# abacus-gene/paml

Measured on AMD Instinct MI355X. Metric: site-patterns/sec per lnL eval (codeml M0, 61 states), higher is better.
Workload: dtype f64; 1 GPU; codeml M0 61-state, 16 taxa x 1000000 synthetic codon patterns sharded over the GPUs (BASELINE configs[3]); classes=1, kernel=mfma64_jit, parallelism=pattern-shard x1, RCCL all-reduce inside the engine, patterns_rank0=1000000

## Files before the change

### include/paml_amd.h

```cpp
#ifndef PAML_AMD_H
#define PAML_AMD_H

#ifdef __cplusplus
extern "C" {
#endif

typedef struct paml_amd_engine paml_amd_engine;

enum {
   PAML_AMD_OK = 0,
   PAML_AMD_EINVAL = -1,
   PAML_AMD_ENOMEM = -2,
   PAML_AMD_EHIP = -3,
   PAML_AMD_EUNSUPPORTED = -4,
   PAML_AMD_ENOCONV = -5
};

enum {
   PAML_AMD_KEEP_PARTIALS = 1,
   PAML_AMD_JIT = 2,
   PAML_AMD_SHARD = 4
};

enum { PAML_AMD_EIGEN_UVROOT = 0, PAML_AMD_EIGEN_CIJK = 1, PAML_AMD_EIGEN_K80 = 2, PAML_AMD_EIGEN_JC69LIKE = 3, PAML_AMD_EIGEN_QMAT = 4 };
// ... 10 lines not shown
#define PAML_AMD_COMM_ID_BYTES 128
int paml_amd_shard_bounds(long n_patt_global, int world, int rank, long *first, long *count);
int paml_amd_max_ranks(long n_patt_global);
int paml_amd_comm_unique_id(void *id128);
int paml_amd_comm_init(paml_amd_engine *e, int rank, int world, const void *id128, long n_patt_global, long first_pattern);
int paml_amd_comm_destroy(paml_amd_engine *e);
int paml_amd_comm_info(const paml_amd_engine *e, int *rank, int *world, long *n_patt_global, long *first_pattern, int *chunk);
int paml_amd_comm_library(char *path, int cap);
int paml_amd_comm_stats(paml_amd_engine *e, int enable, int *n, double *exchange_us_mean, double *exchange_us_max,
                        double *lane_wait_us_mean, double *lane_wait_us_max);

int paml_amd_set_stream(paml_amd_engine *e, void *hip_stream);

int paml_amd_set_tips(paml_amd_engine *e, const unsigned char *z, int cleandata, int n_codes, const int *n_chara,
                      const unsigned char *chara_map, const double *weights, const int *gene_off);

int paml_amd_set_tree(paml_amd_engine *e, int n_nodes, int root, const int *sons_ptr, const int *sons,
                      const int *label, const unsigned char *scale_node);

int paml_amd_set_pi(paml_amd_engine *e, int n_pi, const double *pi);

int paml_amd_set_eigen_qrev_batch(paml_amd_engine *e, int n_sets, const int *set_ids, const double *Q, const double *pi, const double *scale);
int paml_amd_set_eigen_qrev_batch_sparse(paml_amd_engine *e, int n_sets, const int *set_ids, int nnz, const int *row, const int *col,
                                         const double *vals, const double *pi, const double *scale);
int paml_amd_set_eigen_warm_start(paml_amd_engine *e, int on, long *n_warm);
int paml_amd_get_eigen(paml_amd_engine *e, int set_id, double *U, double *V, double *Root);
int paml_amd_eigen_counters(paml_amd_engine *e, long *n_decomposed, int *sweeps_last_batch, int cap);

int paml_amd_set_eigen_uvroot(paml_amd_engine *e, int set_id, const double *U, const double *V, const double *Root);
int paml_amd_set_eigen_cijk(paml_amd_engine *e, int set_id, int nR, const double *Cijk, const double *Root);
int paml_amd_set_eigen_k80(paml_amd_engine *e, int set_id, double kappa);
int paml_amd_set_eigen_jc69like(paml_amd_engine *e, int set_id);
int paml_amd_set_eigen_qmat(paml_amd_engine *e, int set_id, const double *Q);

int paml_amd_set_classes(paml_amd_engine *e, int mode, int K, const double *freqK, const double *rate, int n_labels,
                         const int *eigen_of, const double *qfactor);

int paml_amd_set_gene_class_rates(paml_amd_engine *e, const double *rate);

int paml_amd_eval(paml_amd_engine *e, const double *branch, const double *gene_rate, double *lnL, double *lnf,
                  double *fhK);

int paml_amd_eval_device(paml_amd_engine *e, const double *branch, const double *gene_rate, double *d_lnL);
int paml_amd_flush(paml_amd_engine *e);
int paml_amd_eigen_status(paml_amd_engine *e);

int paml_amd_eval_dirty(paml_amd_engine *e, const double *branch, const double *gene_rate, const unsigned char *clean,
                        double *lnL);

int paml_amd_eval_adg(paml_amd_engine *e, const double *branch, const double *gene_rate, const double *MK, const int *pose, int ls,
                      double *lnL);

int paml_amd_beb_grid(paml_amd_engine *e, int n_grid, int n_cls, const double *pcl, const int *iw, const double *w_class,
                      double *ln_fx, double *pr_last, double *mean_w, double *sd_w);

int paml_amd_beb_grid_classes(paml_amd_engine *e, int n_grid, int n_cls, const double *pcl, const int *iw, double *ln_fx, double *post);

int paml_amd_eval_batch(paml_amd_engine *e, int n_batch, const double *branch, const double *gene_rate, const int *eigen_of,
                        const double *qfactor, const double *freqK, const double *rate, double *lnL, double *lnf);

int paml_amd_eval_branch(paml_amd_engine *e, int node_b, int n_t, const double *t, const double *branch,
                         const double *gene_rate, double *lnL, double *dlnL, double *ddlnL);
int paml_amd_branch_counters(const paml_amd_engine *e, long *n_calls, long *n_nodes_recomputed);
long paml_amd_branch_coef_hits(const paml_amd_engine *e);
long paml_amd_branch_refill_kernels(const paml_amd_engine *e);
double paml_amd_branch_kernel_ms(paml_amd_engine *e);
int paml_amd_get_branch_partials(paml_amd_engine *e, double *out, long cap, long *rows, int *cols);

int paml_amd_node_posterior(paml_amd_engine *e, int node, const double *branch, const double *gene_rate, double *post);

int paml_amd_get_pmat(paml_amd_engine *e, int gene, int iclass, int node, double *P);
int paml_amd_get_partials(paml_amd_engine *e, int node, int iclass, double *conP);
int paml_amd_get_scale(paml_amd_engine *e, int node, int iclass, double *scale);
int paml_amd_get_partial_sums(paml_amd_engine *e, double *out, int cap);

int paml_amd_profile(paml_amd_engine *e, int enable);
int paml_amd_profile_read(paml_amd_engine *e, double *ms_pmat, double *ms_prune, double *ms_reduce, long *n_evals);

int paml_amd_counters(const paml_amd_engine *e, long *n_eval, long *n_pmat);

int paml_amd_cherry_tables(const paml_amd_engine *e, long *n_tabulated, long *bytes);
int paml_amd_subtree_tables(const paml_amd_engine *e, long *n_tabulated, int *nodes, long *u, int cap, long *bytes, long *blocks_left, long *n_computed);
int paml_amd_subtree_order(const paml_amd_engine *e, int *in_use, long *n_computed, double *host_seconds);

int paml_amd_debug_program(int n_tips, int n_nodes, int root, const int *sons_ptr, const int *sons,
                           const unsigned char *scale_node, int keep_partials, const unsigned char *clean,
                           int *ops_out, int cap, int *max_stack);

int paml_amd_debug_branch_plan(int n_tips, int n_nodes, int root, const int *sons_ptr, const int *sons, const unsigned char *scale_node,
                               int n_calls, const int *node_b, const double *branch, int *ends_out, int *up_out, unsigned char *clean_out,
                               int *ops_out, int cap);

int paml_amd_debug_code_order(int n_states, int n_codes, const int *n_chara, const unsigned char *chara_map, const unsigned char *z,
                              long nz, int *order_out);

int paml_amd_debug_jit(int n_tips, int n_nodes, int root, const int *sons_ptr, const int *sons,
                       const unsigned char *scale_node, char *text_out, int cap, int compile);

int paml_amd_debug_jit_tables(int n_tips, int n_nodes, int root, const int *sons_ptr, const int *sons, const unsigned char *scale_node,
                              int max_tabs, char *text_out, int cap, int *stream_out, int stream_cap, int *n_stream, int *tabs_out,
                              int tabs_cap);

int paml_amd_debug_subtree_classes(int n_tips, int n_nodes, int root, const int *sons_ptr, const int *sons, const unsigned char *z, long n_patt,
                                   int n_codes, unsigned int *u_out, unsigned int *cls_out);

int paml_amd_debug_subtree_order(int n_keys, const unsigned int *keys, const unsigned int *bound, long n_patt, int largest_first, int as_given,
                                 unsigned int *order_out);

int paml_amd_debug_subtree_select(int n_tips, int n_nodes, int root, const int *sons_ptr, const int *sons, const unsigned char *scale_node, int n_states,
                                  int n_codes, int K, const unsigned char *z, long n_patt, int *sel_out, int cap);

int paml_amd_debug_jit_subtree(int n_tips, int n_nodes, int root, const int *sons_ptr, const int *sons, const unsigned char *scale_node, int n_states,
                               int n_codes, int K, const int *sel, int n_sel, int compile, const char *dir, char *text_out, int cap, int *blocks_left);

int paml_amd_jit_prebuild(int n_states, int n_tips, int n_codes, int K, long n_patt_global, int n_nodes, int root, const int *sons_ptr,
                          const int *sons, const unsigned char *scale_node, const char *dir, char *log_out, int log_cap);

const char *paml_amd_kernel_name(const paml_amd_engine *e);

int paml_amd_compress_patterns(int n_seq, int n_sites, int width, const unsigned char *chars, const int *gene, int *n_patt,
                               int *first_site, double *weights, int *pose);

int paml_amd_rell_replicates(int n_trees, int n_patt, const double *w, const double *lnf, int n_genes, const int *gene_off, int n_rep,
                             unsigned long long seed, double *rep);
void paml_amd_rell_info(int *chunk, int *tree_block, int *last_batches, double *last_kernel_ms);

int paml_amd_simulate(paml_amd_engine *e, const double *branch, const double *gene_rate, long n_sites, long first_site,
                      unsigned long long seed, unsigned replicate,
                      unsigned char *z ,
                      unsigned char *cls , unsigned char *anc );
void paml_amd_simulate_info(int *last_batches, double *last_kernel_ms);

int paml_amd_ancestral_marginal(paml_amd_engine *e, const double *branch, const double *gene_rate,
                                int n_query, const int *nodes ,
                                unsigned char *best   ,
                                double *best_prob     ,
                                double *post          );

int paml_amd_ancestral_joint(paml_amd_engine *e, const double *branch, const double *gene_rate,
                             unsigned char *states ,
                             double *ln_best       );

void paml_amd_ancestral_info(int *last_batches, double *last_kernel_ms);

int paml_amd_gradient(paml_amd_engine *e, const double *branch, const double *gene_rate, double *lnL,
                      double *grad   ,
                      double *lnf    ,
                      double *scores );
void paml_amd_gradient_info(int *last_batches, double *last_kernel_ms);

int paml_amd_model_gradient(paml_amd_engine *e, const double *branch, const double *gene_rate, double *lnL,
                            double *g_eff   ,
                            double *g_freqK ,
                            double *g_pi    ,
                            double *g_A     ,
                            double *W       );
void paml_amd_model_gradient_info(int *last_batches, double *last_kernel_ms);
int paml_amd_model_gradient_segment(void);
int paml_amd_model_gradient_sizes(paml_amd_engine *e, int *n_pi, int *n_eigen);

int paml_amd_nni_scores(paml_amd_engine *e, const double *branch, const double *gene_rate,
                        int n_swaps, const int *swaps ,
                        double *lnL0, double *lnL , double *lnf );
void paml_amd_nni_info(int *last_batches, double *last_kernel_ms);
int paml_amd_nni_list(int n_tips, int n_nodes, int root, const int *sons_ptr, const int *sons, int *swaps , int cap);

int paml_amd_edge_scores(paml_amd_engine *e, const double *branch, const double *gene_rate,
                         int n_rows, const int *rows ,
                         const int *ovr_node , const double *ovr_t ,
                         double *lnL0, double *lnL, double *d1, double *d2 , double *lnf );
void paml_amd_edge_info(int *last_batches, double *last_kernel_ms);
int paml_amd_edge_list(int n_tips, int n_nodes, int root, const int *sons_ptr, const int *sons,
                       int *edges , int *five , int cap);

int paml_amd_placement_scores(paml_amd_engine *e, const double *branch, const double *gene_rate,
                              int n_q, const unsigned char *qz ,
                              int n_edges, const int *edges ,
                              int n_pend, const double *pendant , double phi, int pendant_label,
                              double *lnL0, double *lnL , double *lnf );
void paml_amd_placement_info(int *last_batches, double *last_kernel_ms);

int paml_amd_spr_scores(paml_amd_engine *e, const double *branch, const double *gene_rate,
                        int n_moves, const int *moves , double phi,
                        double *lnL0, double *lnL , double *lnf );
void paml_amd_spr_info(int *last_batches, double *last_kernel_ms);
int paml_amd_spr_list(int n_tips, int n_nodes, int root, const int *sons_ptr, const int *sons, int radius, int *moves , int cap);

typedef struct paml_amd_pairset paml_amd_pairset;
int paml_amd_pairset_create(paml_amd_engine *e, paml_amd_pairset **out, int n_pairs, const int *seq_a, const int *seq_b);
void paml_amd_pairset_destroy(paml_amd_pairset *ps);
// ... 13 lines not shown
```

### paml_amd/csrc/device_common.h

```cpp
#pragma once
#ifndef __HIPCC_RTC__
#include <hip/hip_runtime.h>
#endif

#include "../../include/paml_amd.h"

namespace paml_amd {

typedef double v4d __attribute__((ext_vector_type(4)));

enum OpCode : int {
   OP_INIT_ONES = 0, OP_INIT_TIP = 1, OP_MUL_TIP = 2, OP_PUSH = 3, OP_MATMUL = 4, OP_MATMUL_POP = 5,
   OP_SCALE = 6, OP_STORE = 7, OP_LOAD = 8, OP_ROOT = 9, OP_END = 10,
   OP_SET_TIP = 11,
   OP_SET_TIP2 = 12,
   OP_MUL_TIP2 = 13,
   OP_EXPORT = 14
};

struct Op { int code, a, b, c; };
__host__ __device__ inline int mm_pop_slot(const Op &o) { return (o.b & 0xff) - 1; }
__host__ __device__ inline int mm_push_slot(const Op &o) { return ((o.b >> 8) & 0xff) - 1; }


struct PruneArgs {
   const Op *ops;
   const unsigned char *z;
   long z_stride;
   const int2 *tiles;
   int n_tiles;
   const int *gene_off;
   const double *weights;
   int n, n_tips, n_nodes, K, n_genes, n_codes, cleandata, n_pi, mode, n_scale, keep, n_patt;
   const double *pi;
   const double *pint;
   const double *ptip;
   double *fhK;
   double *partials;
   double *scalef;
   double *stack_scratch;
   int stack_overflow_slots;
   int first_matmul;
   int n_int;
   int first_tip;
   const void *stream;
   int n_stream;
   long tip_words;
   double *export_buf;
   double *export_scale;
   unsigned long long *prof;
   int prof_stride, prof_tid;
   const double *pcol;
   double *fscale;
   const unsigned char *ztiles;
   int zt_bytes;
   const unsigned int *zpm;
   int zpm_words;
   int Km;
   int chunk;
   int first_chunk, nb_stride;
   int want_fhk;
   const double *freqK;
   long freqK_bs;
   double *lnf;
   double *red_partial;
   double *red_out;
   int *red_counter;
   int nb_local;
   const int *tile_group0;
   int part_groups;
   double *part_dump;
   const unsigned long long *code_mask;
   const double *ctab;
   int n_ctab;
   const double *stab;
   long stab_rows;
   const int *stab_meta;
   const int *order;
};

__device__ __forceinline__ double root_value(const PruneArgs &a, double f, double lnscale)
{
   if (f <= 0) f = (a.mode == PAML_AMD_MODE_LFUN ? 1e-80 : 1e-300);
   if (a.mode == PAML_AMD_MODE_LFUN || a.n_scale) f = log(f) + lnscale;
   return f;
}


typedef double part2_t __attribute__((ext_vector_type(2)));
__device__ __forceinline__ void part_load(const double *p, int lane, double (&x)[16])
{
   const part2_t *p2 = (const part2_t *)p + lane;
#pragma unroll
   for (int i = 0; i < 8; i++) { const part2_t v = p2[i * 64]; x[2 * i] = v.x; x[2 * i + 1] = v.y; }
}
__device__ __forceinline__ void part_store(double *p, int lane, const double (&x)[16])
{
   part2_t *p2 = (part2_t *)p + lane;
#pragma unroll
   for (int i = 0; i < 8; i++) p2[i * 64] = (part2_t){x[2 * i], x[2 * i + 1]};
}
__host__ __device__ inline int part_index(int m, int lane) { return (((m >> 1) * 64 + lane) << 1) | (m & 1); }

#define MFMA_RS 2
#define MFMA_ZT 128

#define CONST_AS __attribute__((address_space(4)))
template <typename T>
__device__ __forceinline__ const CONST_AS T *as_const(const T *p)
{
   return (const CONST_AS T *)(unsigned long long)p;
}
typedef int v4i __attribute__((ext_vector_type(4)));
__device__ __forceinline__ Op fetch_op(const Op *ops, int ip)
{
   const v4i o = ((const CONST_AS v4i *)(unsigned long long)ops)[ip];
   return Op{o.x, o.y, o.z, o.w};
}

typedef __attribute__((address_space(1))) const void gptr_t;
typedef __attribute__((address_space(3))) void lptr_t;

__device__ __forceinline__ __amdgpu_buffer_rsrc_t make_rsrc(const void *base, unsigned bytes)
{
   return __builtin_amdgcn_make_buffer_rsrc((void *)base, 0, bytes, 0x00020000);
}

__device__ __forceinline__ void dma16(__amdgpu_buffer_rsrc_t r, const void *lds, int voff, int soff)
{
   const unsigned la = (unsigned)(unsigned long long)(__attribute__((address_space(3))) const char *)lds;
   asm volatile("s_mov_b32 m0, %0\n\ts_nop 0\n\tbuffer_load_dwordx4 %1, %2, %3 offen lds"
                :
                : "s"(la), "v"(voff), "s"(r), "s"(soff)
                : "memory", "m0");
}

__device__ __forceinline__ void dma4(__amdgpu_buffer_rsrc_t r, const void *lds, int voff, int soff)
{
   const unsigned la = (unsigned)(unsigned long long)(__attribute__((address_space(3))) const char *)lds;
   asm volatile("s_mov_b32 m0, %0\n\ts_nop 0\n\tbuffer_load_dword %1, %2, %3 offen lds"
                :
                : "s"(la), "v"(voff), "s"(r), "s"(soff)
                : "memory", "m0");
}

template <int WAVES>
__device__ __forceinline__ void stage_p(const double *g, double *s, int wave, int lane)
{
   const __amdgpu_buffer_rsrc_t r = make_rsrc(g, 32768);
#pragma unroll
   for (int c = 0; c < 32 / WAVES; c++) {
      const int chunk = c * WAVES + wave;
      dma16(r, (const char *)s + chunk * 1024, lane * 16, chunk * 1024);
   }
}

__device__ __forceinline__ void mfma_matvec(const double *sPbuf, int lane, const double (&cur)[16], v4d (&acc)[4])
{
   const double2 *sp = (const double2 *)sPbuf;
#pragma unroll
   for (int jb = 0; jb < 4; jb++) acc[jb] = (v4d){0, 0, 0, 0};
// ... 1015 lines not shown
```

### paml_amd/csrc/engine_core.hip

```cpp
#include "engine_state.h"
#include "eigen_kernels.h"

namespace paml_amd {
int launch_eigen_qrev(paml_amd_engine *e, EigenQrevArgs a, int n_sets)
{
   if (!e->eigen_attr_set) {
      for (const void *fn : {(const void *)eigen_qrev_kernel<0>, (const void *)eigen_qrev_kernel<20>, (const void *)eigen_qrev_kernel<60>, (const void *)eigen_qrev_kernel<62>})
         HIPCHK(hipFuncSetAttribute(fn, hipFuncAttributeMaxDynamicSharedMemorySize, (int)EIG_LDS_BYTES));
      e->eigen_attr_set = true;
   }
   static const int sweep_limit = getenv("PAML_AMD_EIGEN_SWEEP_LIMIT") ? std::max(1, atoi(getenv("PAML_AMD_EIGEN_SWEEP_LIMIT"))) : 40;
   a.max_sweeps = sweep_limit;
   const int N_even = (a.n + 1) & ~1;
   if (N_even == 62) hipLaunchKernelGGL(eigen_qrev_kernel<62>, dim3(n_sets), dim3(EIG_NT), EIG_LDS_BYTES, e->stream, a);
   else if (N_even == 60) hipLaunchKernelGGL(eigen_qrev_kernel<60>, dim3(n_sets), dim3(EIG_NT), EIG_LDS_BYTES, e->stream, a);
   else if (N_even == 20) hipLaunchKernelGGL(eigen_qrev_kernel<20>, dim3(n_sets), dim3(EIG_NT), EIG_LDS_BYTES, e->stream, a);
   else hipLaunchKernelGGL(eigen_qrev_kernel<0>, dim3(n_sets), dim3(EIG_NT), EIG_LDS_BYTES, e->stream, a);
   HIPCHK(hipGetLastError());
   return 0;
}
}

extern "C" {

// ... 77 lines not shown
{
   enter(e);
   if (!e) return PAML_AMD_EINVAL;
   (void)hipStreamSynchronize(e->stream);
   e->stream = (hipStream_t)hip_stream;
   return 0;
}

int paml_amd_set_tips(paml_amd_engine *e, const unsigned char *z, int cleandata, int n_codes, const int *n_chara,
                      const unsigned char *chara_map, const double *weights, const int *gene_off)
{
   enter(e);
   if (!e || !z || !weights) return fail(e, PAML_AMD_EINVAL, "set_tips: null argument");
   const int n = e->n;
   std::vector<int> nch;
   std::vector<unsigned char> cmap;
   if (cleandata || !n_chara || !chara_map) {
      if (!cleandata) return fail(e, PAML_AMD_EINVAL, "set_tips: cleandata=0 needs n_chara/chara_map");
      n_codes = n;
      nch.assign(n, 1);
      cmap.assign((size_t)n * n, 0);
      for (int i = 0; i < n; i++) cmap[(size_t)i * n] = (unsigned char)i;
   }
   else {
      if (n_codes < 1 || n_codes > 256) return fail(e, PAML_AMD_EINVAL, "set_tips: n_codes out of range");
      nch.assign(n_chara, n_chara + n_codes);
      cmap.assign(chara_map, chara_map + (size_t)n_codes * n);
      for (int c = 0; c < n_codes; c++) {
         if (nch[c] < 0 || nch[c] > n) return fail(e, PAML_AMD_EINVAL, "set_tips: n_chara out of range");
         unsigned long long seen = 0;
         for (int k = 0; k < nch[c]; k++) {
            const int s = cmap[(size_t)c * n + k];
            if (s >= n) return fail(e, PAML_AMD_EINVAL, "set_tips: chara_map state out of range");
            if ((seen >> s) & 1ull) return fail(e, PAML_AMD_EINVAL, "set_tips: a state listed twice in one code's set");
            seen |= 1ull << s;
         }
      }
   }
   const size_t nz = (size_t)e->n_tips * e->n_patt;
   for (size_t i = 0; i < nz; i++)
      if (z[i] >= n_codes) return fail(e, PAML_AMD_EINVAL, "set_tips: character code >= n_codes");
   std::vector<unsigned char> zperm;
   e->code_nch = nch;
   e->code_new_of.resize(n_codes);
   for (int c = 0; c < n_codes; c++) e->code_new_of[c] = (unsigned char)c;
   if (e->kk == KK_MFMA64 && n_codes > 64) {
      std::vector<long> cnt(n_codes, 0);
      for (size_t i = 0; i < nz; i++) cnt[z[i]]++;
      const std::vector<int> order = code_order(n, n_codes, nch.data(), cmap.data(), cnt.data());
      std::vector<unsigned char> new_of(n_codes);
      std::vector<int> nch2(n_codes);
      std::vector<unsigned char> cmap2((size_t)n_codes * n, 0);
      for (int c = 0; c < n_codes; c++) {
         new_of[order[c]] = (unsigned char)c;
         nch2[c] = nch[order[c]];
         memcpy(&cmap2[(size_t)c * n], &cmap[(size_t)order[c] * n], n);
      }
      nch.swap(nch2);
      cmap.swap(cmap2);
      e->code_new_of = new_of;
      zperm.resize(nz);
      for (size_t i = 0; i < nz; i++) zperm[i] = new_of[z[i]];
      z = zperm.data();
   }
   e->amb_ascending = true;
   for (int c = 64; c < n_codes; c++)
      for (int k = 1; k < nch[c]; k++)
         if (cmap[(size_t)c * n + k] <= cmap[(size_t)c * n + k - 1]) e->amb_ascending = false;
   e->cleandata = cleandata ? 1 : 0;
   e->n_codes = n_codes;
   e->plain_codes = 0;
   while (e->plain_codes < std::min(n, n_codes) && nch[e->plain_codes] == 1 && cmap[(size_t)e->plain_codes * n] == e->plain_codes) e->plain_codes++;
   e->gene_off.assign(e->n_genes + 1, 0);
   if (gene_off) e->gene_off.assign(gene_off, gene_off + e->n_genes + 1);
   else {
      if (e->n_genes != 1) return fail(e, PAML_AMD_EINVAL, "set_tips: gene_off required when n_genes > 1");
      e->gene_off[1] = e->n_patt;
   }
   if (e->gene_off[0] != 0 || e->gene_off[e->n_genes] != e->n_patt)
      return fail(e, PAML_AMD_EINVAL, "set_tips: gene_off must span [0, n_patt]");
   for (int g = 0; g < e->n_genes; g++)
      if (e->gene_off[g + 1] < e->gene_off[g]) return fail(e, PAML_AMD_EINVAL, "set_tips: gene_off must not decrease");
   HIPCHK(upload(e->d_z, z, nz, e->stream));
   if (e->kk == KK_MFMA64 && e->n_genes == 1 && n_codes <= 64) e->h_z.assign(z, z + nz);
   else std::vector<unsigned char>().swap(e->h_z);
   e->tips_gen++;
   HIPCHK(upload(e->d_weights, weights, (size_t)e->n_patt, e->stream));
   HIPCHK(upload(e->d_n_chara, nch.data(), nch.size(), e->stream));
   HIPCHK(upload(e->d_chara_map, cmap.data(), cmap.size(), e->stream));
   HIPCHK(upload(e->d_gene_off, e->gene_off.data(), e->gene_off.size(), e->stream));
   if (e->kk == KK_VALU4 || e->kk == KK_VALU5 || e->kk == KK_VALU20) {
      e->zpm_words = ((e->n_tips + 3) / 4 + 3) / 4 * 4;
      HIPCHK(e->d_zpm.ensure((size_t)e->n_patt * e->zpm_words));
      launch_zpm(e->d_z.p, (long)e->n_patt, e->n_tips, e->n_patt, e->zpm_words, e->d_zpm.p, e->stream);
   }
   HIPCHK(hipStreamSynchronize(e->stream));
   e->tile_stash.built_for = 0;
   int r = build_tiles(e);
   if (r) return r;
   {
      std::vector<unsigned long long> mask(n_codes, 0);
      for (int c = 0; c < n_codes; c++)
         for (int k = 0; k < nch[c]; k++) mask[c] |= 1ull << cmap[(size_t)c * n + k];
      HIPCHK(upload(e->d_code_mask, mask.data(), mask.size(), e->stream));
      HIPCHK(hipStreamSynchronize(e->stream));
   }
   e->have_tips = true;
   e->partials_valid = false;
   e->bl.valid = false;
   return 0;
}

int paml_amd_set_tree(paml_amd_engine *e, int n_nodes, int root, const int *sons_ptr, const int *sons, const int *label,
                      const unsigned char *scale_node)
{
   enter(e);
   if (!e || !sons_ptr || !sons) return fail(e, PAML_AMD_EINVAL, "set_tree: null argument");
   if (n_nodes <= e->n_tips || root < 0 || root >= n_nodes) return fail(e, PAML_AMD_EINVAL, "set_tree: bad sizes");
   TreeDesc t;
   t.n_tips = e->n_tips; t.n_nodes = n_nodes; t.root = root;
   t.sons_ptr.assign(sons_ptr, sons_ptr + n_nodes + 1);
   if (t.sons_ptr[0] != 0) return fail(e, PAML_AMD_EINVAL, "set_tree: sons_ptr[0] != 0");
   for (int i = 0; i < n_nodes; i++)
      if (t.sons_ptr[i + 1] < t.sons_ptr[i]) return fail(e, PAML_AMD_EINVAL, "set_tree: sons_ptr not monotone");
   t.sons.assign(sons, sons + t.sons_ptr[n_nodes]);
   std::vector<int> seen(n_nodes, 0);
   for (int s : t.sons) {
      if (s < 0 || s >= n_nodes || s == root || seen[s]++) return fail(e, PAML_AMD_EINVAL, "set_tree: bad son index");
   }
   for (int i = 0; i < n_nodes; i++) {
      if (i != root && !seen[i]) return fail(e, PAML_AMD_EINVAL, "set_tree: node without father");
      if (i >= e->n_tips && t.is_leaf(i)) return fail(e, PAML_AMD_EINVAL, "set_tree: internal node without sons");
      if (i < e->n_tips && i != root && !t.is_leaf(i)) return fail(e, PAML_AMD_EINVAL, "set_tree: tip with sons");
   }
   t.label.assign(n_nodes, 0);
   if (label) t.label.assign(label, label + n_nodes);
   t.scale_node.assign(n_nodes, 0);
   t.scale_slot.assign(n_nodes, -1);
   if (scale_node) {
      for (int i = 0; i < n_nodes; i++) {
         t.scale_node[i] = scale_node[i] ? 1 : 0;
         if (t.scale_node[i]) t.scale_slot[i] = t.n_scale++;
      }
   }
   std::vector<unsigned char> leaf(n_nodes);
   for (int i = 0; i < n_nodes; i++) leaf[i] = t.is_leaf(i) ? 1 : 0;
   e->tree = std::move(t);
   e->tree_gen++;
   HIPCHK(upload(e->d_label, e->tree.label.data(), e->tree.label.size(), e->stream));
   HIPCHK(upload(e->d_is_leaf, leaf.data(), leaf.size(), e->stream));
   HIPCHK(hipStreamSynchronize(e->stream));
   e->have_tree = true;
   e->pres_valid = false;
   e->prog_valid = false;
   e->partials_valid = false;
   e->bl.valid = false;
   return 0;
}

int paml_amd_set_pi(paml_amd_engine *e, int n_pi, const double *pi)
{
   enter(e);
   if (!e || !pi || (n_pi != 1 && n_pi != e->n_genes)) return fail(e, PAML_AMD_EINVAL, "set_pi: bad arguments");
   const int n = e->n;
   std::vector<double> buf;
   if (e->kk == KK_MFMA64) {
      buf.assign((size_t)n_pi * 64, 0.0);
      for (int g = 0; g < n_pi; g++)
// ... 402 lines not shown
         for (int hl = 0; hl < 16; hl++) {
            const int h = tiles[t].y + w * 16 + hl;
            if (h >= hend) continue;
            const double *grp = raw.data() + (t * MW + w) * 1024;
            for (int j = 0; j < n; j++) conP[(size_t)h * n + j] = grp[part_index(j >> 2, (j & 3) * 16 + hl)];
         }
   }
   return 0;
}

int paml_amd_get_scale(paml_amd_engine *e, int node, int iclass, double *scale)
{
   enter(e);
   if (!e || !scale) return fail(e, PAML_AMD_EINVAL, "get_scale: null argument");
   if (!(e->flags & PAML_AMD_KEEP_PARTIALS) || !e->partials_valid)
      return fail(e, PAML_AMD_EINVAL, "get_scale: needs PAML_AMD_KEEP_PARTIALS and a completed evaluation");
   if (node < 0 || node >= e->tree.n_nodes || iclass < 0 || iclass >= e->K || e->tree.scale_slot[node] < 0)
      return fail(e, PAML_AMD_EINVAL, "get_scale: not a scaling node");
   const double *src = e->d_scalef.p + ((size_t)iclass * e->tree.n_scale + e->tree.scale_slot[node]) * e->n_patt;
   HIPCHK(hipMemcpyAsync(scale, src, (size_t)e->n_patt * sizeof(double), hipMemcpyDeviceToHost, e->stream));
   HIPCHK(hipStreamSynchronize(e->stream));
   return 0;
}

int paml_amd_profile(paml_amd_engine *e, int enable)
{
   if (!e) return PAML_AMD_EINVAL;
   enter(e);
   e->profiling = enable != 0;
   return 0;
}

int paml_amd_profile_read(paml_amd_engine *e, double *ms_pmat, double *ms_prune, double *ms_reduce, long *n_evals)
{
   if (!e) return PAML_AMD_EINVAL;
   HIPCHK(hipStreamSynchronize(e->stream));
   double acc[3] = {0, 0, 0};
   for (size_t i = 0; i + 5 < e->ev_used.size(); i += 6)
      for (int k = 0; k < 3; k++) {
         float ms = 0;
         if (hipEventElapsedTime(&ms, e->ev_used[i + 2 * k], e->ev_used[i + 2 * k + 1]) == hipSuccess) acc[k] += ms;
      }
   for (auto ev : e->ev_used) e->ev_pool.push_back(ev);
   e->ev_used.clear();
   if (ms_pmat) *ms_pmat = acc[0];
   if (ms_prune) *ms_prune = acc[1];
   if (ms_reduce) *ms_reduce = acc[2];
   if (n_evals) *n_evals = e->prof_evals;
   e->prof_evals = 0;
   return 0;
}

int paml_amd_cherry_tables(const paml_amd_engine *e, long *n_tabulated, long *bytes)
{
   if (!e) return PAML_AMD_EINVAL;
   if (n_tabulated) *n_tabulated = e->last_ctab_n;
   if (bytes) *bytes = e->last_ctab_bytes;
   return 0;
}

int paml_amd_subtree_tables(const paml_amd_engine *e, long *n_tabulated, int *nodes, long *u, int cap, long *bytes, long *blocks_left, long *n_computed)
{
   if (!e) return PAML_AMD_EINVAL;
   if (n_tabulated) *n_tabulated = e->last_stab_n;
   for (long i = 0; i < e->last_stab_n && i < cap && i < (long)e->sub.sel.size(); i++) {
      if (nodes) nodes[i] = e->sub.sel[i];
      if (u) u[i] = (long)e->sub.u[e->sub.sel[i]];
   }
   if (bytes) *bytes = e->last_stab_bytes;
   if (blocks_left) *blocks_left = e->last_stab_blocks;
   if (n_computed) *n_computed = e->sub.n_computed;
   return 0;
}

int paml_amd_subtree_order(const paml_amd_engine *e, int *in_use, long *n_computed, double *host_seconds)
{
   if (!e) return PAML_AMD_EINVAL;
   if (in_use) *in_use = (e->last_stab_n && e->sub.ordered) ? 1 : 0;
   if (n_computed) *n_computed = e->sub.n_order_computed;
   if (host_seconds) *host_seconds = e->sub.order_host_s;
   return 0;
}

int paml_amd_counters(const paml_amd_engine *e, long *n_eval, long *n_pmat)
{
   if (!e) return PAML_AMD_EINVAL;
   if (n_eval) *n_eval = e->n_eval;
   if (n_pmat) *n_pmat = e->n_pmat;
   return 0;
}

}
```

### paml_amd/csrc/engine_eval.hip

```cpp
#include "engine_state.h"
#include "kernels_pmat.h"
#include "kernels_prune.h"
#include "kernels_reduce.h"

namespace paml_amd {

int build_tiles(paml_amd_engine *e)
{
   std::vector<int2> tiles;
   for (int g = 0; g < e->n_genes; g++)
      for (int h = e->gene_off[g]; h < e->gene_off[g + 1]; h += e->tile_patt) tiles.push_back(make_int2(g, h));
   e->n_tiles = (int)tiles.size();
   HIPCHK(upload(e->d_tiles, tiles.data(), tiles.size(), e->stream));
   const int tf = e->kk == KK_MFMA64 ? GATHER_WAVES * 16 : 256;
   std::vector<int2> tfull;
   for (int g = 0; g < e->n_genes; g++)
      for (int h = e->gene_off[g]; h < e->gene_off[g + 1]; h += tf) tfull.push_back(make_int2(g, h));
   e->n_tiles_full = (int)tfull.size();
   HIPCHK(upload(e->d_tiles_full, tfull.data(), tfull.size(), e->stream));
   if (e->kk == KK_MFMA64) {
      std::vector<int> g0(tiles.size());
      size_t k = 0;
      int base = 0;
      for (int g = 0; g < e->n_genes; g++) {
// ... 339 lines not shown
      sb.level_first.push_back((int)by_level.size());
      int tiles = 0;
      bool tip_son = false;
      for (int i = 0; i < ns; i++)
         if (sb.sp.sub[i].level == l) {
            by_level.push_back(i);
            tiles = std::max(tiles, (int)((sb.u[sb.sp.sub[i].node] + 127) / 128));
            tip_son = tip_son || sb.sp.sub[i].l.kind == 0 || sb.sp.sub[i].r.kind == 0;
         }
      sb.level_tiles.push_back(tiles);
      sb.level_small.push_back(tip_son ? 0 : 1);
   }
   sb.level_first.push_back((int)by_level.size());
   sb.rowmap.assign(ns, std::vector<unsigned int>());
   std::vector<std::vector<unsigned int>> son_rows(ns);
   for (int i = 0; i < ns; i++) {
      const SubtreeTab &st = sb.sp.sub[i];
      const size_t u = sb.u[st.node];
      const std::vector<unsigned int> &sc = sb.son_cls[st.node];
      std::vector<unsigned int> l(sc.begin(), sc.begin() + u), r(sc.begin() + u, sc.end());
      if (st.l.kind == 2 && !sb.rowmap[st.l.id].empty()) for (unsigned int &x : l) x = sb.rowmap[st.l.id][x];
      if (st.r.kind == 2 && !sb.rowmap[st.r.id].empty()) for (unsigned int &x : r) x = sb.rowmap[st.r.id][x];
      son_rows[i].resize(2 * u);
      if (e->env.subtree_rows) {
         std::vector<unsigned int> by(u);
         for (size_t c = 0; c < u; c++) by[c] = (unsigned int)c;
         std::sort(by.begin(), by.end(), [&](unsigned int a, unsigned int b) { return l[a] != l[b] ? l[a] < l[b] : (r[a] != r[b] ? r[a] < r[b] : a < b); });
         sb.rowmap[i].resize(u);
         for (size_t row = 0; row < u; row++) { sb.rowmap[i][by[row]] = (unsigned int)row; son_rows[i][row] = l[by[row]]; son_rows[i][u + row] = r[by[row]]; }
      }
      else { std::copy(l.begin(), l.end(), son_rows[i].begin()); std::copy(r.begin(), r.end(), son_rows[i].begin() + u); }
   }
   std::vector<SubtreeNodeDev> nodes(ns);
   std::vector<unsigned int> sidx;
   for (int k = 0; k < ns; k++) {
      const SubtreeTab &st = sb.sp.sub[by_level[k]];
      SubtreeNodeDev &nd = nodes[k];
      nd.node = st.node; nd.u = (int)sb.u[st.node]; nd.row0 = row0[by_level[k]];
      nd.lkind = st.l.kind; nd.lid = st.l.kind == 2 ? row0[st.l.id] : st.l.id;
      nd.rkind = st.r.kind; nd.rid = st.r.kind == 2 ? row0[st.r.id] : st.r.id;
      nd.pad = 0;
      nd.sidx = (long)sidx.size();
      sidx.insert(sidx.end(), son_rows[by_level[k]].begin(), son_rows[by_level[k]].end());
   }
   std::vector<int> meta;
   for (int ti : sb.sp.top) { meta.push_back(row0[ti]); meta.push_back((int)sb.u[sb.sp.sub[ti].node]); }
   HIPCHK(upload(sb.d_nodes, nodes.data(), nodes.size(), e->stream));
   HIPCHK(upload(sb.d_sidx, sidx.data(), sidx.size(), e->stream));
   HIPCHK(upload(sb.d_meta, meta.data(), meta.size(), e->stream));
   HIPCHK(hipStreamSynchronize(e->stream));
   return 0;
}

int ensure_subtree_ztiles(paml_amd_engine *e)
{
   paml_amd_engine::Subtree &sb = e->sub;
   if (sb.zt_sel_gen == sb.sel_gen && sb.zt_tiles == e->n_tiles && sb.zt_tile_patt == e->tile_patt) return 0;
   const int n_top = (int)sb.sp.top.size();
   std::vector<unsigned int> top((size_t)n_top * e->n_patt);
   for (int k = 0; k < n_top; k++) {
      const std::vector<unsigned int> &c = sb.cls[sb.sp.sub[sb.sp.top[k]].node], &rm = sb.rowmap[sb.sp.top[k]];
      if (rm.empty()) std::copy(c.begin(), c.end(), top.begin() + (size_t)k * e->n_patt);
      else for (long h = 0; h < e->n_patt; h++) top[(size_t)k * e->n_patt + h] = rm[c[h]];
   }
   sb.ordered = e->env.subtree_order != 0;
   if (sb.ordered && sb.order_sel_gen != sb.sel_gen) {
      const auto t0 = std::chrono::steady_clock::now();
      std::vector<const unsigned int *> keys;
      std::vector<unsigned int> bound;
      for (int k = 0; k < n_top; k++) { keys.push_back(top.data() + (size_t)k * e->n_patt); bound.push_back(sb.u[sb.sp.sub[sb.sp.top[k]].node]); }
      std::vector<std::vector<unsigned int>> cherry_cls;
      for (const Op &o : sb.sp.prog.ops)
         if (o.code == OP_LOOKUP && o.c < SUBTREE_TAB_BASE) {
            const CherryTab &ct = sb.sp.tabs[o.c];
            const unsigned char *za = e->h_z.data() + (size_t)ct.tip_a * e->n_patt, *zb = e->h_z.data() + (size_t)ct.tip_b * e->n_patt;
            cherry_cls.emplace_back(e->n_patt);
            for (long h = 0; h < e->n_patt; h++) cherry_cls.back()[h] = (unsigned int)za[h] * e->n_codes + zb[h];
         }
      for (const std::vector<unsigned int> &c : cherry_cls) { keys.push_back(c.data()); bound.push_back((unsigned int)(e->n_codes * e->n_codes)); }
      const std::vector<unsigned int> order = subtree_pattern_order(keys, bound, subtree_order_sequence(bound, e->env.subtree_order == 2), (long)e->n_patt);
      sb.order_host_s = std::chrono::duration<double>(std::chrono::steady_clock::now() - t0).count();
      HIPCHK(upload(sb.d_order, (const int *)order.data(), order.size(), e->stream));
      HIPCHK(hipStreamSynchronize(e->stream));
      sb.order_sel_gen = sb.sel_gen;
      sb.n_order_computed++;
   }
   sb.zt_bytes = jit_zpieces(jit_subtree_zrows(e->n_tips, n_top), e->tile_patt) * 2048;
   HIPCHK(upload(sb.d_top_cls, top.data(), top.size(), e->stream));
   HIPCHK(sb.d_ztiles.ensure((size_t)e->n_tiles * sb.zt_bytes));
   hipLaunchKernelGGL(sztile_kernel, dim3(e->n_tiles), dim3(e->tile_patt), 0, e->stream, e->d_tiles.p, e->d_gene_off.p, e->d_z.p, (long)e->n_patt, e->d_weights.p,
                      e->n_tips, sb.zt_bytes, sb.d_ztiles.p, n_top, sb.d_top_cls.p, sb.ordered ? sb.d_order.p : nullptr);
   HIPCHK(hipStreamSynchronize(e->stream));
   sb.d_top_cls.release();
   sb.zt_sel_gen = sb.sel_gen; sb.zt_tiles = e->n_tiles; sb.zt_tile_patt = e->tile_patt;
   return 0;
}

int choose_kernel(paml_amd_engine *e, const Eval &c, PruneKernel *out)
{
   const int n = e->n, Km = c.Km, G = c.G;
   if (e->kk == KK_MFMA64) {
      bool lean = e->prog.max_stack <= MFMA_RS && e->n_tips <= MFMA_ZT && e->n_codes <= 64;
      if ((e->n_patt + 127) / 128 <= e->n_cu / 4) lean = false;
      for (const Op &o : e->prog.ops)
         if (o.code == OP_PUSH || o.code == OP_SCALE || o.code == OP_STORE || o.code == OP_LOAD) lean = false;
      bool jit_ok = false;
      const int jw = 8;
      bool has_load = false;
      for (const Op &o : e->prog.ops) has_load = has_load || o.code == OP_LOAD;
      e->n_ctab = 0;
      e->n_stab = 0;
      if (e->jit_enabled && !(has_load && e->n_tips > 207) && (e->n_codes <= 64 || (e->amb_ascending && e->plain_codes >= n)) && jit_supported(e->prog, e->n_tips, e->n_codes, e->n_pi, 6, jw * 16, true)) {
         const std::string pkey = jit_program_key(e->prog, e->n_tips);
         std::string key = "m" + std::to_string(n) + "c" + std::to_string(e->n_codes) + "w" + std::to_string(jw) + ":" + pkey;
         int n_tab = 0;
         if (e->env.cherry_tables != 0 && G == 1 && e->n_pi == 1 && c.B == 1 && !c.keep && !c.clean && !has_load &&
             (e->env.cherry_tables == 1 || e->n_patt >= e->env.cherry_min_patt)) {
            const std::string ckey = ckey_of(e, c.K, n, pkey);
            if (e->cherry_key != ckey) {
               e->cherry_n = jit_cherry_count(e->prog, e->n_tips, n, e->n_codes, c.K, (size_t)e->env.cherry_cap_mb << 20, jw * 16);
               e->cherry = e->cherry_n ? jit_cherry_program(e->prog, e->cherry_n) : CherryProgram();
               e->cherry_key = ckey;
               e->cherry_gen++;
            }
            n_tab = e->cherry_n;
         }
         if (n_tab && e->env.subtree_tables != 0) {
            if (int r = ensure_subtree(e, c.K, jw * 16)) return r;
            if (!e->sub.sel.empty()) {
               std::string skey = "s";
               for (int v : e->sub.sel) skey += std::to_string(v) + ".";
               skey += "t" + std::to_string(n_tab) + key;
               const bool ordered = e->env.subtree_order != 0;
               if (ordered) skey = "o" + skey;
               bool ok = false;
               const int n_top = (int)e->sub.sp.top.size();
               if (int r = obtain_kernel(e, e->jit_slot, &e->jit, true, skey, [&]() { return jit_generate(e->sub.sp.prog, e->n_tips, n, e->n_codes, &e->sub.sp.tabs, n_top, ordered); },
                                         (e->prog.ops.size() > 120 && !e->jit_forced && !e->env.jit_sync) ? JIT_WAIT_WORKER : JIT_WAIT_CALLER, "tree, subtree tables", &ok)) return r;
               if (ok) { jit_ok = true; e->n_ctab = n_tab; e->n_stab = (int)e->sub.sel.size(); }
            }
         }
         if (n_tab && !jit_ok) {
            const std::string tkey = "t" + std::to_string(n_tab) + key;
            bool ok = false;
            if (int r = obtain_kernel(e, e->jit_slot, &e->jit, true, tkey, [&]() { return jit_generate(e->cherry.prog, e->n_tips, n, e->n_codes, &e->cherry.tabs); },
                                      (e->prog.ops.size() > 120 && !e->jit_forced && !e->env.jit_sync) ? JIT_WAIT_WORKER : JIT_WAIT_CALLER, "tree, cherry tables", &ok)) return r;
            if (ok) { jit_ok = true; e->n_ctab = n_tab; }
         }
         const bool big = e->prog.ops.size() > 120;
         const bool background = (big || has_load) && !e->jit_forced && !e->env.jit_sync;
         const bool wanted = !has_load || e->jit_forced || e->env.jit_sync || e->jit_recall(key) || e->jit_count_request(key) >= 2;
         if (wanted && !jit_ok)
            if (int r = obtain_kernel(e, e->jit_slot, &e->jit, true, key, [&]() { return jit_generate(e->prog, e->n_tips, n, e->n_codes); },
                                      background ? JIT_WAIT_WORKER : JIT_WAIT_CALLER, "tree", &jit_ok)) return r;
      }
      const bool big_tiles = jit_ok || lean;
      const int want_waves = jit_ok ? jw : (lean ? DMA_WAVES : GATHER_WAVES);
      if (int r = select_tiles(e, big_tiles, want_waves, jit_ok)) return r;
      if (e->n_stab)
         if (int r = ensure_subtree_ztiles(e)) return r;
      if (jit_ok || e->mfma_dma) {
         *out = jit_ok ? PK_MFMA64_JIT : PK_MFMA64_STREAM;
         return 0;
      }
      bool coop = !c.keep && !c.clean && !e->env.no_coop && e->tile_patt == 64 && e->prog.max_stack <= COOP_SLOTS &&
                  (long)e->n_tiles * 4 * c.K <= (long)e->n_cu && !e->env.prof_ops.size();
      bool coopj = false;
      for (const Op &o : e->prog.ops) coop = coop && o.code != OP_STORE && o.code != OP_LOAD && o.code != OP_EXPORT;
      if (coop && e->coopj_enabled && !e->comm && e->nb_global == (e->n_patt + e->chunk - 1) / e->chunk && e->first_chunk == 0 &&
          jit_coop_supported(e->prog, e->n_tips, e->n_codes)) {
         const std::string key = "cj" + std::to_string(n <= 32 ? n : 64) + ":" + jit_program_key(e->prog, e->n_tips);
         if (int r = obtain_kernel(e, e->coop_slot, &e->jit_coop, false, key, [&]() { return jit_generate_coop(e->prog, e->n_tips, n); },
                                   (e->jit_forced || e->env.jit_sync) ? JIT_WAIT_CALLER : JIT_WAIT_WORKER, "coop", &coopj)) return r;
      }
      *out = coopj ? PK_MFMA64_COOPJIT : (coop ? PK_MFMA64_COOP : PK_MFMA64_GATHER);
      return 0;
   }
   bool jit_ok = false, second = false;
   if (e->jit_enabled && !c.keep && n <= 5 && jit_valu_supported(e->prog)) {
      const ValuFusedPlan pl = jit_valu_fused_plan(e->prog, n, e->n_tips, e->n_codes, Km, e->chunk);
      const bool vf_genes = getenv("PAML_AMD_VF_GENES") && atoi(getenv("PAML_AMD_VF_GENES")) != 0;
      if (pl.ok && (G == 1 ? e->n_pi == 1 : (vf_genes && (e->n_pi == 1 || e->n_pi == G))) && e->d_zpm.p && G <= 64) {
         int r = obtain_kernel(e, e->jit_slot, &e->jit, true, std::string("vf") + std::to_string(n) + "c" + std::to_string(e->n_codes) + "k" + std::to_string(Km) + "r" + std::to_string(pl.R) + "w" +
                                     std::to_string(pl.CW) + (pl.cherry ? "y" : "n") + (G > 1 ? "g" + std::to_string(G) + ":" : ":") + jit_program_key(e->prog, e->n_tips),
                               [&]() { return jit_generate_valu_fused(e->prog, n, e->n_tips, e->n_codes, Km, e->chunk, G); }, JIT_WAIT_CALLER, "valu fused", &jit_ok);
         if (r) return r;
         second = jit_ok;
         e->fused_threads = 256 * pl.CW;
      }
      if (!jit_ok) {
         int r = obtain_kernel(e, e->jit_slot, &e->jit, true, "v" + std::to_string(n) + ":" + jit_program_key(e->prog, e->n_tips),
                               [&]() { return jit_generate_valu(e->prog, n); }, JIT_WAIT_CALLER, "valu", &jit_ok);
         if (r) return r;
      }
   }
   if (e->want_m20 && !c.clean && jit_m20_supported(e->prog, e->n_tips, G)) {
      int r = obtain_kernel(e, e->jit_slot, &e->jit, true, std::string("m20c") + std::to_string(e->n_codes) + (G > 1 ? "g:" : ":") + jit_program_key(e->prog, e->n_tips),
                            [&]() { return jit_generate_m20(e->prog, e->n_tips, e->n_codes, G > 1 ? 2 : 1); }, JIT_WAIT_CALLER, "m20", &jit_ok);
      if (r) return r;
      second = jit_ok;
   }
   *out = PruneKernel(3 * e->kk + (second ? 2 : (jit_ok ? 1 : 0)));
   return 0;
}

int ensure_buffers(paml_amd_engine *e, Eval &c)
{
   if (c.pipe) {
      paml_amd_engine::PSet &sp = e->spare[e->spare_head];
      std::swap(e->d_rowmajor, sp.rowmajor); std::swap(e->d_pint, sp.pint); std::swap(e->d_ptip, sp.ptip); std::swap(e->d_pcol, sp.pcol);
      std::swap(e->d_ctab, sp.ctab);
      std::swap(e->d_stab, sp.stab);
      std::swap(e->pset, sp.id);
      e->spare_head = (e->spare_head + 1) % (paml_amd_engine::NPSET - 1);
   }
   if (int rc = ensure_pmat_buffers(e, c.psets, e->kk == KK_VALU20 && e->want_m20, e->kk == KK_MFMA64)) return rc;
   if (e->kernel != PK_MFMA64_JIT) e->n_ctab = e->n_stab = 0;
   e->last_stab_n = e->n_stab;
   e->last_stab_bytes = e->n_stab ? (long)((size_t)c.K * e->sub.rows * CHERRY_ROW_BYTES) : 0;
   e->last_stab_blocks = e->n_stab ? (long)(e->sub.sp.prog.stream.size() / 2) : -1;
   if (e->n_stab) HIPCHK(e->d_stab.ensure((size_t)e->last_stab_bytes / sizeof(double)));
   e->last_ctab_n = e->n_ctab;
   e->last_ctab_bytes = (long)((size_t)c.K * e->n_ctab * cherry_table_bytes(e->n_codes));
   if (e->n_ctab) HIPCHK(e->d_ctab.ensure((size_t)e->last_ctab_bytes / sizeof(double)));
   HIPCHK(e->d_fhK.ensure((size_t)c.K * e->n_patt));
   c.n_blocks = e->n_tiles * c.K;
   if (c.keep) {
      const int n_int = e->tree.n_nodes - e->n_tips;
      size_t words = e->kk == KK_MFMA64 ? (size_t)c.K * n_int * e->part_groups() * 1024 + (size_t)std::max(e->mfma_waves, 8) * 1024
                                        : (size_t)c.K * n_int * e->n_patt * e->n;
      HIPCHK(e->d_partials.ensure(words));
      HIPCHK(e->d_scalef.ensure((size_t)c.K * std::max(1, e->tree.n_scale) * e->n_patt));
   }
   return stack_overflow(e, e->prog, c.n_blocks, e->mfma_waves, &c.overflow);
}

int run_pmat(paml_amd_engine *e, Eval &c, const InlineVec &iv)
{
   const int B = c.B, Km = c.Km, G = c.G, nn = e->tree.n_nodes;
   const BatchSpec *const bs = c.bs;
   PmatArgs pa = pmat_args(e, e->tree.root, e->d_label.p, e->kk == KK_MFMA64 ? 1 : (e->kernel == PK_MFMA4X20_JIT ? 2 : 0),
                           e->kk == KK_MFMA64 ? e->d_pcol.p : nullptr);
   if (c.pipe) { pa.branch = e->d2_branch.p; pa.gene_rate = e->d2_gene_rate.p; }
// ... 69 lines not shown
   }
   mark_on(e, c.ps);
   if (c.pipe) {
      HIPCHK(hipEventRecord(e->ev_pmat, e->s2));
      HIPCHK(hipStreamWaitEvent(c.ms, e->ev_pmat, 0));
   }
   if (c.want_pipe && !c.skip_entry) {
      HIPCHK(hipEventRecord(e->ev_entry[e->entry_sel], c.ms));
      e->entry_sel ^= 1;
      e->have_prev_entry = true;
   }
   e->n_pmat += (long)c.psets * (nn - 1);
   return 0;
}

int wait_slot(paml_amd_engine *e, Eval &c)
{
   if (c.slot_waited) return 0;
   c.slot_waited = true;
   if (e->done_pending[c.slot]) {
      e->done_pending[c.slot] = false;
      if (c.ms != e->stream || e->join_pending[c.slot]) {
         const int si = (int)(e->st_count % paml_amd_engine::NSTAT);
         if (e->comm_stats) HIPCHK(hipEventRecord(e->st_w0[si], c.ms));
         HIPCHK(hipStreamWaitEvent(c.ms, e->ev_done[c.slot], 0));
         if (e->comm_stats) { HIPCHK(hipEventRecord(e->st_w1[si], c.ms)); e->st_waited[si] = true; }
         if (c.ms == e->stream) e->join_pending[c.slot] = false;
      }
   }
   return 0;
}

int prepare_slot(paml_amd_engine *e, Eval &c)
{
   const int B = c.B, nbg = e->nb_global;
   c.offload = c.want_pipe && !pk_forms_reduction(e->kernel) && !c.keep && !c.clean && !c.bs && !c.want_lnf && !e->tree.n_scale && e->env.offload;
   c.side_total = e->comm || c.dual;
   if (!c.offload && !c.side_total)
      if (int rc = join_comm(e)) return rc;
   c.slot = (c.side_total || c.offload) ? e->red_slot : 0;
   if (e->comm_stats && !e->st_part[0])
      for (int i = 0; i < paml_amd_engine::NSTAT; i++) {
         HIPCHK(hipEventCreate(&e->st_part[i])); HIPCHK(hipEventCreate(&e->st_done[i]));
         HIPCHK(hipEventCreate(&e->st_w0[i])); HIPCHK(hipEventCreate(&e->st_w1[i]));
      }
   if (e->comm_stats) e->st_waited[e->st_count % paml_amd_engine::NSTAT] = false;
   DevBuf<double> &dpart = e->part_slot(c.slot);
   if ((size_t)nbg * B > dpart.cap) {
      if (e->sc) HIPCHK(hipStreamSynchronize(e->sc));
      HIPCHK(dpart.ensure((size_t)nbg * B));
      HIPCHK(hipMemsetAsync(dpart.p, 0, dpart.cap * sizeof(double), c.ms));
   }
   e->last_fhk = (c.offload || c.dual) ? c.slot : 0;
   if (e->last_fhk) HIPCHK(e->fhk_slot(e->last_fhk).ensure((size_t)c.K * e->n_patt));
   c.slot_waited = false;
   if (c.offload) {
      if (int rc = ensure_side_stream(e)) return rc;
      if (int rc = wait_slot(e, c)) return rc;
   }
   if ((size_t)B * RED_TICKET_WORDS > e->d_red_counter.cap) {
      HIPCHK(e->d_red_counter.ensure((size_t)std::max(B, 64) * RED_TICKET_WORDS));
      HIPCHK(hipMemsetAsync(e->d_red_counter.p, 0, e->d_red_counter.cap * sizeof(int), c.ms));
   }
   HIPCHK(e->d_out.ensure(B));
   if (c.want_lnf) HIPCHK(e->d_lnf.ensure((size_t)B * e->n_patt));
   return 0;
}

int run_prune(paml_amd_engine *e, Eval &c)
{
   const PruneKernel k = e->kernel;
   const int B = c.B, K = c.K, G = c.G, n_blocks = c.n_blocks;
   const BatchSpec *const bs = c.bs;
   if (pk_module(k) && e->tree.n_scale) HIPCHK(e->d_fscale.ensure((size_t)K * e->n_patt));
   PruneArgs pr = prune_args(e, e->prog, K, e->d_ops.p, false, e->tree.n_scale, c.keep, e->d_partials.p, e->d_scalef.p, c.overflow);
   if (k == PK_MFMA4X20_JIT) { pr.pint = e->d_pint.p; pr.pcol = e->d_rowmajor.p; }
   pr.fhK = e->fhk_slot(e->last_fhk).p;
   if (k == PK_MFMA64_JIT && e->n_ctab) { pr.ctab = e->d_ctab.p; pr.n_ctab = e->n_ctab; }
   if (k == PK_MFMA64_JIT && e->n_stab) {
      pr.stab = e->d_stab.p; pr.stab_rows = e->sub.rows; pr.stab_meta = e->sub.d_meta.p;
      pr.ztiles = e->sub.d_ztiles.p; pr.zt_bytes = e->sub.zt_bytes;
      pr.order = e->sub.ordered ? e->sub.d_order.p : nullptr;
   }
   const int nb = (e->n_patt + e->chunk - 1) / e->chunk;
   if (pk_forms_reduction(k)) {
      pr.Km = c.Km; pr.chunk = e->chunk; pr.first_chunk = e->first_chunk; pr.nb_stride = e->nb_global;
      pr.want_fhk = (c.want_fhk || e->tree.n_scale) ? 1 : 0;
      pr.freqK = (bs && bs->freqK) ? e->d_b_freqK.p : e->d_freqK.p; pr.freqK_bs = (bs && bs->freqK) ? c.Km : 0;
      pr.lnf = c.want_lnf ? e->d_lnf.p : nullptr;
      pr.red_partial = e->part_slot(c.slot).p; pr.red_out = c.d_lnL_out ? c.d_lnL_out : e->d_out.p; pr.nb_local = nb;
      if (int rc = wait_slot(e, c)) return rc;
      pr.red_counter = k == PK_MFMA64_COOPJIT ? e->d_red_counter.p : nullptr;
   }
   if (!e->env.prof_ops.empty()) {
      const int prof_stride = std::max((int)e->prog.ops.size() + 3, e->env.prof_tiles ? 96 : 0);
      const size_t words = (size_t)3 * n_blocks * prof_stride;
      if (!e->env.prof_tiles || words != e->prof_words) {
         if (e->d_prof) (void)hipFree(e->d_prof);
         e->d_prof = nullptr;
         HIPCHK(hipMalloc((void **)&e->d_prof, paml_amd_engine::MAXL * words * 8));
         HIPCHK(hipMemsetAsync(e->d_prof, 0, paml_amd_engine::MAXL * words * 8, c.ms));
         e->prof_words = words; e->prof_blocks = n_blocks; e->prof_stride = prof_stride;
      }
      pr.prof = e->d_prof + (size_t)c.lane * words;
      pr.prof_stride = prof_stride;
      pr.prof_tid = e->env.prof_tid;
   }
   mark(e);
   const bool two_streams = c.want_pipe && e->env.dual && !e->profiling;
   const int cus = (e->comm && !two_streams) ? std::max(1, e->n_cu - e->comm_cus) : e->n_cu;
   void *params[] = {&pr};
   hipStream_t const ms = c.ms;
   switch (k) {
   case PK_MFMA64_JIT:
      HIPCHK(hipModuleLaunchKernel(e->jit.fn, std::min(n_blocks, cus), 1, 1, e->mfma_waves * 64, 1, 1, 0, ms, params, nullptr));
      break;
   case PK_MFMA64_STREAM:
      if (!e->stream_attr_set) {
         HIPCHK(hipFuncSetAttribute((const void *)prune_mfma64_stream, hipFuncAttributeMaxDynamicSharedMemorySize, 160 * 1024));
         e->stream_attr_set = true;
      }
      hipLaunchKernelGGL(prune_mfma64_stream, dim3(n_blocks), dim3(512), (size_t)4 * 4096 * sizeof(double) + (size_t)e->n_tips * 128, ms, pr);
      break;
   case PK_MFMA64_COOPJIT:
      HIPCHK(hipModuleLaunchKernel(e->jit_coop.fn, e->n_tiles * 4 * K, 1, 1, 256, 1, 1, 0, ms, params, nullptr));
      break;
   case PK_MFMA64_COOP:
      hipLaunchKernelGGL(prune_mfma64_coop, dim3(e->n_tiles * 4 * K), dim3(256), 0, ms, pr);
      break;
   case PK_VALU4_FUSED_JIT: case PK_VALU5_FUSED_JIT: {
      const int gx = B > 1 ? std::max(1, std::min(nb, 2 * e->n_cu / B)) : nb;
      HIPCHK(hipModuleLaunchKernel(e->jit.fn, gx, B, 1, e->fused_threads, 1, 1, 0, ms, params, nullptr));
      break;
   }
   case PK_MFMA4X20_JIT: {
      int grid = std::min(std::max(K, cus / K * K), e->n_tiles * K);
      if (two_streams && G == 1) {
         const int units = std::min(e->n_tiles * 8, (e->n_patt + 31) / 32), g78 = e->n_cu * 7 / 8 / K * K;
         auto rounds = [&](int g) { return ((units + g / K - 1) / (g / K) + 7) / 8; };
         if (g78 >= K && g78 < grid && rounds(g78) == rounds(grid)) grid = g78;
      }
      HIPCHK(hipModuleLaunchKernel(e->jit.fn, std::max(grid / K, G > 1 ? G : 1) * K, 1, 1, 512, 1, 1, 0, ms, params, nullptr));
      break;
   }
   case PK_VALU4_JIT: case PK_VALU5_JIT: case PK_VALU20_JIT:
      HIPCHK(hipModuleLaunchKernel(e->jit.fn, n_blocks, 1, 1, 256, 1, 1, 0, ms, params, nullptr));
      break;
   case PK_MFMA64_GATHER: case PK_VALU4: case PK_VALU5: case PK_VALU20:
      launch_prune_full(e, e->prog.max_stack, n_blocks, pr, ms);
      break;
   }
   mark(e);
   if (c.want_pipe && e->env.dual) {
      HIPCHK(hipEventRecord(e->ev_setread[e->pset], ms));
      e->setread_rec[e->pset] = true;
   }
   return 0;
}

int dump_op_stamps(paml_amd_engine *e, const Eval &c)
{
   if (e->env.prof_ops.empty() || e->env.prof_tiles) return 0;
   std::vector<unsigned long long> hp((size_t)3 * e->prof_blocks * e->prof_stride);
   HIPCHK(hipMemcpyAsync(hp.data(), e->d_prof, hp.size() * 8, hipMemcpyDeviceToHost, c.ms));
   HIPCHK(hipStreamSynchronize(c.ms));
   if (FILE *f = fopen(e->env.prof_ops.c_str(), "wb")) {
      int hdr[2] = {e->prof_blocks, e->prof_stride};
      fwrite(hdr, sizeof(int), 2, f);
      std::vector<int> codes;
      for (auto &o : e->prog.ops) codes.push_back(o.code);
      codes.resize(e->prof_stride - 3, 0);
      fwrite(codes.data(), sizeof(int), codes.size(), f);
      fwrite(hp.data(), 8, hp.size(), f);
      fclose(f);
   }
   return 0;
}

int reduce(paml_amd_engine *e, Eval &c)
{
   const PruneKernel k = e->kernel;
   const int B = c.B, Km = c.Km, slot = c.slot, nbg = e->nb_global, nb = (e->n_patt + e->chunk - 1) / e->chunk;
   const BatchSpec *const bs = c.bs;
   DevBuf<double> &dpart = e->part_slot(slot);
   ReduceArgs ra{};
   ra.fhK = e->fhk_slot(e->last_fhk).p; ra.weights = e->d_weights.p; ra.freqK = e->d_freqK.p; ra.lnf = c.want_lnf ? e->d_lnf.p : nullptr;
   ra.partial = dpart.p; ra.out = c.d_lnL_out ? c.d_lnL_out : e->d_out.p;
   ra.raw = pk_leaves_log(k) ? 1 : 0; ra.fscale = e->d_fscale.p;
   ra.n_patt = e->n_patt; ra.K = Km; ra.mode = e->mode; ra.n_scale = e->tree.n_scale; ra.chunk = e->chunk;
   ra.first_chunk = e->first_chunk; ra.nb_stride = nbg;
   if (bs && bs->freqK) { ra.freqK = e->d_b_freqK.p; ra.freqK_bs = Km; }
   hipStream_t rs = c.ms;
   if (c.offload) {
      HIPCHK(hipEventRecord(e->ev_part[slot], c.ms));
      HIPCHK(hipStreamWaitEvent(e->sc, e->ev_part[slot], 0));
      rs = e->sc;
   }
// ... 214 lines not shown
```

### paml_amd/csrc/engine_jitdbg.hip

```cpp
#include "engine_state.h"

static int prebuild_genes() { const char *v = getenv("PAML_AMD_PREBUILD_GENES"); return v && atoi(v) > 1 ? atoi(v) : 1; }

static bool tree_from_csr(int n_tips, int n_nodes, int root, const int *sons_ptr, const int *sons, const unsigned char *scale_node, TreeDesc *out)
{
   if (!sons_ptr || !sons || n_nodes <= 0 || root < 0 || root >= n_nodes) return false;
   TreeDesc &t = *out;
   t.n_tips = n_tips; t.n_nodes = n_nodes; t.root = root;
   t.sons_ptr.assign(sons_ptr, sons_ptr + n_nodes + 1);
   t.sons.assign(sons, sons + sons_ptr[n_nodes]);
   t.label.assign(n_nodes, 0);
   t.scale_node.assign(n_nodes, 0);
   t.scale_slot.assign(n_nodes, -1);
   if (scale_node)
      for (int i = 0; i < n_nodes; i++)
         if (scale_node[i]) { t.scale_node[i] = 1; t.scale_slot[i] = t.n_scale++; }
   return true;
}

extern "C" {

int paml_amd_debug_program(int n_tips, int n_nodes, int root, const int *sons_ptr, const int *sons,
                           const unsigned char *scale_node, int keep_partials, const unsigned char *clean,
                           int *ops_out, int cap, int *max_stack)
// ... 93 lines not shown
   }
   else if (n_states == 4 || n_states == 5 || n_states == 20) {
      if (!jit_valu_supported(p)) return PAML_AMD_EUNSUPPORTED;
      text = jit_generate_valu(p, n_states);
   }
   else {
      if (!jit_supported(p, n_tips, 61)) return PAML_AMD_EUNSUPPORTED;
      text = jit_generate(p, n_tips, 61, 64);
   }
   int rc = (int)text.size();
   if (compile) {
      std::vector<char> code;
      std::string log;
      if (jit_compile_code(text, &code, &log, getenv("PAML_AMD_JIT_SHIP")) != 0) {
         text = log;
         rc = PAML_AMD_EHIP;
      }
   }
   if (text_out && cap > 0) {
      const size_t ncp = std::min((size_t)cap - 1, text.size());
      memcpy(text_out, text.data(), ncp);
      text_out[ncp] = 0;
   }
   return rc;
}

int paml_amd_debug_jit_tables(int n_tips, int n_nodes, int root, const int *sons_ptr, const int *sons, const unsigned char *scale_node,
                              int max_tabs, char *text_out, int cap, int *stream_out, int stream_cap, int *n_stream, int *tabs_out, int tabs_cap)
{
   TreeDesc t;
   if (!tree_from_csr(n_tips, n_nodes, root, sons_ptr, sons, scale_node, &t)) return PAML_AMD_EINVAL;
   const Program p = build_program(t, false, nullptr);
   if (!jit_supported(p, n_tips, 61)) return PAML_AMD_EUNSUPPORTED;
   const int n_tab = jit_cherry_count(p, n_tips, 61, 61, 1, (size_t)std::max(max_tabs, 0) * cherry_table_bytes(61));
   if (n_stream) *n_stream = 0;
   if (text_out && cap > 0) text_out[0] = 0;
   if (!n_tab) return 0;
   const CherryProgram cp = jit_cherry_program(p, n_tab);
   const std::string text = jit_generate(cp.prog, n_tips, 61, 61, &cp.tabs);
   if (text_out && cap > 0) {
      const size_t ncp = std::min((size_t)cap - 1, text.size());
      memcpy(text_out, text.data(), ncp);
      text_out[ncp] = 0;
   }
   if (n_stream) *n_stream = (int)cp.prog.stream.size() / 2;
   if (stream_out)
      for (int i = 0; i < (int)cp.prog.stream.size() && i < stream_cap; i++) stream_out[i] = cp.prog.stream[i];
   if (tabs_out)
      for (int i = 0; i < n_tab && 3 * i + 2 < tabs_cap; i++) { tabs_out[3 * i] = cp.tabs[i].tip_a; tabs_out[3 * i + 1] = cp.tabs[i].tip_b; tabs_out[3 * i + 2] = cp.tabs[i].node; }
   return n_tab;
}

int paml_amd_debug_subtree_classes(int n_tips, int n_nodes, int root, const int *sons_ptr, const int *sons, const unsigned char *z, long n_patt,
                                   int n_codes, unsigned int *u_out, unsigned int *cls_out)
{
   TreeDesc t;
   if (!z || n_patt < 1 || n_codes < 1 || !tree_from_csr(n_tips, n_nodes, root, sons_ptr, sons, nullptr, &t)) return PAML_AMD_EINVAL;
   for (long i = 0; i < (long)n_tips * n_patt; i++)
      if (z[i] >= n_codes) return PAML_AMD_EINVAL;
   const SubtreeClasses sc = subtree_classes(n_tips, n_nodes, root, t.sons_ptr.data(), t.sons.data(), z, n_patt, n_patt, n_codes);
   for (int v = 0; v < n_nodes; v++) {
      if (u_out) u_out[v] = sc.u[v];
      if (cls_out && sc.done[v]) memcpy(cls_out + (long)v * n_patt, sc.cls[v].data(), (size_t)n_patt * sizeof(unsigned int));
   }
   return 0;
}

int paml_amd_debug_subtree_order(int n_keys, const unsigned int *keys, const unsigned int *bound, long n_patt, int largest_first, int as_given,
                                 unsigned int *order_out)
{
   if (n_keys < 0 || n_patt < 1 || (n_keys && (!keys || !bound)) || !order_out) return PAML_AMD_EINVAL;
   std::vector<const unsigned int *> k(n_keys);
   std::vector<unsigned int> b(n_keys);
   std::vector<int> seq(n_keys);
   for (int i = 0; i < n_keys; i++) { k[i] = keys + (long)i * n_patt; b[i] = bound[i]; seq[i] = i; }
   for (long i = 0; i < (long)n_keys * n_patt; i++)
      if (keys[i] >= bound[i / n_patt]) return PAML_AMD_EINVAL;
   if (!as_given) seq = subtree_order_sequence(b, largest_first != 0);
   const std::vector<unsigned int> order = subtree_pattern_order(k, b, seq, n_patt);
   memcpy(order_out, order.data(), (size_t)n_patt * sizeof(unsigned int));
   return 0;
}

int paml_amd_debug_subtree_select(int n_tips, int n_nodes, int root, const int *sons_ptr, const int *sons, const unsigned char *scale_node, int n_states,
                                  int n_codes, int K, const unsigned char *z, long n_patt, int *sel_out, int cap)
{
   TreeDesc t;
   if (!z || n_patt < 1 || !tree_from_csr(n_tips, n_nodes, root, sons_ptr, sons, scale_node, &t)) return PAML_AMD_EINVAL;
   const Program p = build_program(t, false, nullptr);
   if (!jit_supported(p, n_tips, n_codes)) return 0;
   EnvCfg env;
   env.read();
   const int n_tab = env.subtree_tables != 0 ? jit_cherry_count(p, n_tips, n_states, n_codes, K, (size_t)env.cherry_cap_mb << 20) : 0;
   if (!n_tab) return 0;
   const CherryProgram cp = jit_cherry_program(p, n_tab);
   const double lim_u = env.subtree_max_frac * (double)n_patt;
   const SubtreeClasses sc = subtree_classes(n_tips, n_nodes, root, t.sons_ptr.data(), t.sons.data(), z, n_patt, n_patt, n_codes,
                                             lim_u >= 4e9 ? ~0ull : (uint64_t)std::max(0.0, lim_u));
   const std::vector<int> sel = jit_subtree_select(t, cp.tabs, sc.u, sc.done, n_patt, env.subtree_max_frac, (size_t)env.subtree_cap_mb << 20, K);
   for (int i = 0; i < (int)sel.size() && i < cap; i++)
      if (sel_out) sel_out[i] = sel[i];
   return (int)sel.size();
}

int paml_amd_debug_jit_subtree(int n_tips, int n_nodes, int root, const int *sons_ptr, const int *sons, const unsigned char *scale_node, int n_states,
                               int n_codes, int K, const int *sel, int n_sel, int compile, const char *dir, char *text_out, int cap, int *blocks_left)
{
   TreeDesc t;
   if (!sel || n_sel < 1 || !tree_from_csr(n_tips, n_nodes, root, sons_ptr, sons, scale_node, &t)) return PAML_AMD_EINVAL;
   const Program p = build_program(t, false, nullptr);
   if (!jit_supported(p, n_tips, n_codes)) return PAML_AMD_EUNSUPPORTED;
   EnvCfg env;
   env.read();
   const int n_tab = jit_cherry_count(p, n_tips, n_states, n_codes, K, (size_t)env.cherry_cap_mb << 20);
   if (text_out && cap > 0) text_out[0] = 0;
   if (!n_tab) return 0;
   const CherryProgram cp = jit_cherry_program(p, n_tab);
   std::vector<unsigned int> u(n_nodes, 0);
   std::vector<char> done(n_nodes, 0);
   for (int i = 0; i < n_sel; i++) {
      if (sel[i] < n_tips || sel[i] >= n_nodes) return PAML_AMD_EINVAL;
      u[sel[i]] = 1 + i;
      done[sel[i]] = 1;
   }
   const std::vector<int> ok = jit_subtree_select(t, cp.tabs, u, done, 1L << 30, 1.0, ~(size_t)0 >> 8, 1);
   if ((int)ok.size() != n_sel) return 0;
   const SubtreeProgram sp = jit_subtree_program(p, n_tab, t, ok);
   if (sp.top.empty() || !jit_subtree_zfits(n_tips, (int)sp.top.size())) return 0;
   if (blocks_left) *blocks_left = (int)sp.prog.stream.size() / 2;
   std::string text = jit_generate(sp.prog, n_tips, n_states, n_codes, &sp.tabs, (int)sp.top.size(), env.subtree_order != 0);
   int rc = (int)text.size();
   if (compile) {
      std::vector<char> code;
      std::string log;
      if (jit_compile_code(text, &code, &log, (dir && *dir) ? dir : nullptr) != 0) {
         text = log;
         rc = PAML_AMD_EHIP;
      }
   }
   if (text_out && cap > 0) {
      const size_t ncp = std::min((size_t)cap - 1, text.size());
      memcpy(text_out, text.data(), ncp);
      text_out[ncp] = 0;
   }
   return rc;
}

int paml_amd_jit_prebuild(int n_states, int n_tips, int n_codes, int K, long n_patt_global, int n_nodes, int root, const int *sons_ptr,
                          const int *sons, const unsigned char *scale_node, const char *dir, char *log_out, int log_cap)
{
   TreeDesc t;
   if (!dir || n_states < 2 || n_states > 64 || !tree_from_csr(n_tips, n_nodes, root, sons_ptr, sons, scale_node, &t)) return PAML_AMD_EINVAL;
   const Program p = build_program(t, n_states > 20 && getenv("PAML_AMD_PREBUILD_KEEP") != nullptr, nullptr);
   std::string text;
   if (getenv("PAML_AMD_PREBUILD_COOP")) {
      if (!jit_coop_supported(p, n_tips, n_codes)) return PAML_AMD_EUNSUPPORTED;
      text = jit_generate_coop(p, n_tips, n_states);
   }
   else if (n_states == 20 && jit_m20_supported(p, n_tips, prebuild_genes())) text = jit_generate_m20(p, n_tips, n_codes, prebuild_genes());
   else if (n_states <= 5) {
      if (!jit_valu_supported(p)) return PAML_AMD_EUNSUPPORTED;
      const int chunk = red_chunk(n_patt_global);
      text = !jit_valu_fused_plan(p, n_states, n_tips, n_codes, K, chunk).ok ? jit_generate_valu(p, n_states)
                                                                               : jit_generate_valu_fused(p, n_states, n_tips, n_codes, K, chunk, prebuild_genes());
   }
   else {
// ... 30 lines not shown
```

### paml_amd/csrc/engine_state.h

```cpp
#pragma once
#include <hip/hip_runtime.h>

#include <algorithm>
#include <cmath>
#include <cstdio>
#include <cstdlib>
#include <cstring>
#include <string>
#include <atomic>
#include <functional>
#include <memory>
#include <mutex>
#include <set>
#include <thread>
#include <vector>

#include <dlfcn.h>
#include <unistd.h>
#include <rccl/rccl.h>

#include "../../include/paml_amd.h"
#include "jit.h"
#include "jit_cache.h"
#include "kernel_args.h"
#include "program.h"
#include "branch_plan.h"
#include "subtree_classes.h"

namespace paml_amd {
static_assert(JIT_SCRATCH_BASE == MFMA_RS, "the per-tree kernel addresses the interpreter's overflow-stack scratch");

enum KernelKind { KK_VALU4, KK_VALU5, KK_VALU20, KK_MFMA64 };
enum PruneKernel {
   PK_VALU4, PK_VALU4_JIT, PK_VALU4_FUSED_JIT, PK_VALU5, PK_VALU5_JIT, PK_VALU5_FUSED_JIT, PK_VALU20, PK_VALU20_JIT, PK_MFMA4X20_JIT,
   PK_MFMA64_JIT, PK_MFMA64_STREAM, PK_MFMA64_COOP, PK_MFMA64_COOPJIT, PK_MFMA64_GATHER
};
inline bool pk_module(PruneKernel k) { return k == PK_MFMA64_JIT || (k < PK_MFMA64_JIT && k % 3 != 0); }
inline bool pk_forms_reduction(PruneKernel k) { return k == PK_VALU4_FUSED_JIT || k == PK_VALU5_FUSED_JIT || k == PK_MFMA64_COOPJIT; }
inline bool pk_leaves_log(PruneKernel k) { return k == PK_MFMA64_JIT || k == PK_MFMA4X20_JIT; }
inline bool pk_persistent(PruneKernel k) { return k == PK_MFMA64_JIT || k == PK_MFMA4X20_JIT; }
constexpr int DMA_WAVES = 8;
constexpr int GATHER_WAVES = 4;
constexpr int VALU_MAXD_SMALL = 16, VALU_MAXD_20 = 8;

template <typename T>
struct DevBuf {
   T *p = nullptr;
   size_t cap = 0;
   hipError_t ensure(size_t n)
   {
      if (n <= cap) return hipSuccess;
      if (p) (void)hipFree(p);
      p = nullptr;
      cap = 0;
      hipError_t e = hipMalloc((void **)&p, std::max<size_t>(n, 1) * sizeof(T));
      if (e == hipSuccess) cap = n;
      return e;
   }
   void release()
   {
      if (p) (void)hipFree(p);
      p = nullptr;
      cap = 0;
   }
};

struct Staging {
   char *p = nullptr;
   size_t cap = 0, used = 0;
   hipEvent_t ev = nullptr;
   bool pending = false;
   hipError_t begin(size_t need)
   {
      if (pending) { hipError_t r = hipEventSynchronize(ev); if (r != hipSuccess) return r; pending = false; }
      if (need > cap) {
         if (p) (void)hipHostFree(p);
         p = nullptr; cap = 0;
         hipError_t r = hipHostMalloc((void **)&p, need * 2, hipHostMallocDefault);
         if (r != hipSuccess) return r;
         cap = need * 2;
      }
      if (!ev) { hipError_t r = hipEventCreateWithFlags(&ev, hipEventDisableTiming); if (r != hipSuccess) return r; }
      used = 0;
      return hipSuccess;
   }
   template <typename T>
   T *put(const T *src, size_t n)
   {
      used = (used + 15) & ~(size_t)15;
      T *dst = (T *)(p + used);
      memcpy(dst, src, n * sizeof(T));
      used += n * sizeof(T);
      return dst;
   }
   template <typename T>
   hipError_t send(DevBuf<T> &b, const T *src, size_t n, hipStream_t s)
   {
      const hipError_t r = b.ensure(n);
      return r != hipSuccess ? r : hipMemcpyAsync(b.p, put(src, n), n * sizeof(T), hipMemcpyHostToDevice, s);
   }
   hipError_t end(hipStream_t s) { pending = true; return hipEventRecord(ev, s); }
   void release()
   {
      if (pending && ev) (void)hipEventSynchronize(ev);
      if (p) (void)hipHostFree(p);
      if (ev) (void)hipEventDestroy(ev);
      p = nullptr; ev = nullptr; cap = 0; pending = false;
   }
};

struct EigenHost {
   int kind = -1, nR = 0;
   double kappa = 0;
   DevBuf<double> U, V, Root, Cijk;
   DevBuf<double> Rt[2];
   int rt_cur = 0;
   int warm_run = -1;
   unsigned long long live_mask = 0;
   double sig[8] = {0, 0, 0, 0, 0, 0, 0, 0};
};

struct Rccl {
   void *h = nullptr;
   decltype(&ncclGetUniqueId) GetUniqueId = nullptr;
   decltype(&ncclCommInitRank) CommInitRank = nullptr;
   decltype(&ncclCommDestroy) CommDestroy = nullptr;
   decltype(&ncclAllReduce) AllReduce = nullptr;
   decltype(&ncclGetErrorString) GetErrorString = nullptr;
   std::string err;
   bool load()
   {
      if (h) return true;
      const char *names[] = {getenv("PAML_AMD_RCCL_LIB"), "librccl.so.1", "/opt/rocm/lib/librccl.so.1", "librccl.so"};
      for (const char *nm : names)
         if (nm && *nm && (h = dlopen(nm, RTLD_NOW | RTLD_GLOBAL))) break;
      if (!h) { err = std::string("dlopen librccl.so.1: ") + dlerror(); return false; }
      GetUniqueId = (decltype(GetUniqueId))dlsym(h, "ncclGetUniqueId");
      CommInitRank = (decltype(CommInitRank))dlsym(h, "ncclCommInitRank");
      CommDestroy = (decltype(CommDestroy))dlsym(h, "ncclCommDestroy");
      AllReduce = (decltype(AllReduce))dlsym(h, "ncclAllReduce");
      GetErrorString = (decltype(GetErrorString))dlsym(h, "ncclGetErrorString");
      if (!GetUniqueId || !CommInitRank || !CommDestroy || !AllReduce || !GetErrorString) {
         err = "librccl.so.1 lacks an expected symbol";
         h = nullptr;
         return false;
      }
      return true;
   }
};
inline Rccl &rccl()
{
   static Rccl r;
   return r;
}

inline int red_chunk(long n_global) { return (int)std::max<long>(256, ((n_global + 1023) / 1024 + 255) / 256 * 256); }

struct EnvCfg {
   bool offload = false;
   bool dual = true;
   bool no_coef_cache = false;
   bool no_branch_eig = false;
   bool no_coop = false;
   bool jit_sync = false, jit_strict = false, no_m20 = false;
   int comm_cus = -1, lanes = 0;
   int cherry_tables = -1;
   long cherry_min_patt = 32768, cherry_cap_mb = 192;
   int subtree_tables = -1;
   double subtree_max_frac = 0.5;
   long subtree_cap_mb = 2048;
   int subtree_order = 1;
   int subtree_rows = 1;
   std::string jit_dump, prof_ops;
   int prof_tid = 0;
   bool prof_tiles = false;
   bool comm_stats = false;
   void read()
   {
      if (const char *v = getenv("PAML_AMD_COOP")) no_coop = atoi(v) == 0;
      offload = getenv("PAML_AMD_OFFLOAD") != nullptr;
      if (const char *v = getenv("PAML_AMD_DUAL")) dual = atoi(v) != 0;
      jit_sync = getenv("PAML_AMD_JIT_SYNC") != nullptr;
      jit_strict = getenv("PAML_AMD_JIT_STRICT") != nullptr;
      no_m20 = getenv("PAML_AMD_NO_M20") != nullptr;
      no_branch_eig = getenv("PAML_AMD_NO_BRANCH_EIG") != nullptr;
      no_coef_cache = getenv("PAML_AMD_NO_COEF_CACHE") != nullptr;
      if (const char *v = getenv("PAML_AMD_COMM_CUS")) comm_cus = atoi(v);
      comm_stats = getenv("PAML_AMD_COMM_STATS") != nullptr;
      if (const char *v = getenv("PAML_AMD_LANES")) lanes = atoi(v);
      if (const char *v = getenv("PAML_AMD_CHERRY_TABLES")) cherry_tables = atoi(v) != 0 ? 1 : 0;
      if (const char *v = getenv("PAML_AMD_CHERRY_MIN_PATT")) cherry_min_patt = atol(v);
      if (const char *v = getenv("PAML_AMD_CHERRY_CAP_MB")) cherry_cap_mb = std::max(0L, atol(v));
      if (const char *v = getenv("PAML_AMD_SUBTREE_TABLES")) subtree_tables = atoi(v) != 0 ? 1 : 0;
      if (const char *v = getenv("PAML_AMD_SUBTREE_MAX_FRAC")) subtree_max_frac = std::max(0.0, atof(v));
      if (const char *v = getenv("PAML_AMD_SUBTREE_CAP_MB")) subtree_cap_mb = std::max(0L, atol(v));
      if (const char *v = getenv("PAML_AMD_SUBTREE_ORDER")) subtree_order = std::max(0, std::min(2, atoi(v)));
      if (const char *v = getenv("PAML_AMD_SUBTREE_ROWS")) subtree_rows = atoi(v) != 0 ? 1 : 0;
      if (const char *v = getenv("PAML_AMD_JIT_DUMP")) jit_dump = v;
      if (const char *v = getenv("PAML_AMD_PROF_OPS")) prof_ops = v;
      if (const char *v = getenv("PAML_AMD_PROF_TID")) prof_tid = atoi(v);
      prof_tiles = getenv("PAML_AMD_PROF_TILES") != nullptr;
   }
};

}

using namespace paml_amd;

inline void worker_threads_list(std::thread *th, bool add)
{
   static std::mutex m;
   static std::vector<std::pair<std::thread *, pid_t>> live;
   static const bool registered = (atexit([]() { worker_threads_list(nullptr, false); }), true);
   (void)registered;
   std::vector<std::thread *> to_join;
   {
      std::lock_guard<std::mutex> lk(m);
      if (th && add) live.emplace_back(th, getpid());
      else if (th) live.erase(std::remove_if(live.begin(), live.end(), [th](const std::pair<std::thread *, pid_t> &e) { return e.first == th; }), live.end());
      else
         for (const auto &e : live)
            if (e.second == getpid()) to_join.push_back(e.first);
   }
   for (std::thread *t : to_join)
      if (t->joinable()) t->join();
}

struct paml_amd_engine {
   int n = 0, n_tips = 0, n_patt = 0, max_classes = 0, n_genes = 1;
   unsigned flags = 0;
   KernelKind kk = KK_MFMA64;
   PruneKernel kernel = PK_MFMA64_STREAM;
   bool mfma_dma = true;
   int mfma_waves = DMA_WAVES;
   int tile_patt = 64;
   hipStream_t stream = nullptr;
   std::string err;
   EnvCfg env;
   int device = 0, n_cu = 0;
   bool stream_attr_set = false;
   unsigned long long *d_prof = nullptr;
   size_t prof_words = 0;
   int prof_blocks = 0, prof_stride = 0;

   ncclComm_t comm = nullptr;
   int rank = 0, world = 1;
   long n_patt_global = 0, first_patt = 0;
   int chunk = 256, nb_global = 1, first_chunk = 0;
   DevBuf<double> d_partial_tot, d_btot;
   hipStream_t sc = nullptr;
   static constexpr int MAXL = 4;
   int n_lanes = 2;
   hipEvent_t ev_part[MAXL] = {}, ev_done[MAXL] = {};
   bool done_pending[MAXL] = {}, join_pending[MAXL] = {};
   static constexpr int NSTAT = 64;
   bool comm_stats = false;
   hipEvent_t st_part[NSTAT] = {}, st_done[NSTAT] = {}, st_w0[NSTAT] = {}, st_w1[NSTAT] = {};
   bool st_waited[NSTAT] = {};
   long st_count = 0;
   int red_slot = 0, last_slot = 0, last_fhk = 0;
   int comm_cus = 2;
   DevBuf<double> d_partial_s[MAXL - 1], d_partial_tot_s[MAXL - 1], d_fhK_s[MAXL - 1];
   DevBuf<double> &part_slot(int b) { return b ? d_partial_s[b - 1] : d_partial; }
   DevBuf<double> &tot_slot(int b) { return b ? d_partial_tot_s[b - 1] : d_partial_tot; }
   DevBuf<double> &fhk_slot(int b) { return b ? d_fhK_s[b - 1] : d_fhK; }
   DevBuf<unsigned int> d_zpm;
   int zpm_words = 0;
   DevBuf<int> d_red_counter;
   long bpart_rows = 0; int bpart_cols = 0;
   bool bpart_colmajor = false;
   double *h_out = nullptr;
   size_t h_out_cap = 0;
   bool rate_per_gene = false;
   std::vector<double> class_rate;
   bool want_m20 = false;
   int fused_threads = 256;
   bool pmat_valid = false;
   BranchCache bl;
   DevBuf<double> d_bl_partials, d_bl_scalef, d_bl_frag, d_bl_coef, d_bl_efrag, d_bl_ztab, d_bl_etab, d_bl_ecol;
   bool beig_attr_set = false;
// ... 2 lines not shown
   bool bk_timed = false;
   long n_branch_coef_hits = 0;
   long n_branch_refill_jit = 0;
   DevBuf<unsigned long long> d_code_mask;
   long n_branch_eval = 0, n_branch_nodes = 0;

   bool have_tips = false, have_tree = false, have_pi = false, have_classes = false;
   int cleandata = 1, n_codes = 0;
   std::vector<int> code_nch;
   std::vector<unsigned char> code_new_of;
   DevBuf<unsigned char> d_z, d_chara_map, d_is_leaf, d_ztiles;
   int zt_bytes = 0;
   DevBuf<int> d_n_chara, d_gene_off, d_label, d_eigen_of, d_b_eigen_of;
   DevBuf<int2> d_tiles, d_tiles_full;
   int n_tiles_full = 0;
   DevBuf<int> d_ztip_of;
   std::string zt_key;
   DevBuf<int> d_tile_group0;
   struct TileStash {
      int built_for = 0;
      int n_tiles = 0, zt_bytes = 0;
      std::string zt_key;
      DevBuf<int2> tiles;
      DevBuf<int> group0, ztip_of;
      DevBuf<unsigned char> ztiles;
   } tile_stash;
   int tiles_built_for = 0;
   void swap_tile_stash()
   {
      TileStash &t = tile_stash;
      std::swap(t.built_for, tiles_built_for); std::swap(t.n_tiles, n_tiles); std::swap(t.zt_bytes, zt_bytes); std::swap(t.zt_key, zt_key);
      std::swap(t.tiles, d_tiles); std::swap(t.group0, d_tile_group0); std::swap(t.ztip_of, d_ztip_of); std::swap(t.ztiles, d_ztiles);
   }
   int part_groups() const { return n_tiles_full * GATHER_WAVES; }
   DevBuf<double> d_pi_plain;
   DevBuf<double> d_weights, d_pi, d_freqK, d_rate, d_qfactor, d_branch, d_gene_rate;
   std::vector<int> gene_off;
   int n_tiles = 0, n_pi = 1;

   TreeDesc tree;
   Program prog;
   bool prog_valid = false;
   DevBuf<Op> d_ops;
   DevBuf<int> d_stream;
   Staging stage;
   JitKernel jit;
   CherryProgram cherry;
   std::string cherry_key;
   int cherry_n = 0;
   DevBuf<double> d_ctab;
   int n_ctab = 0;
   bool ctab_attr_set = false;
   long last_ctab_n = 0, last_ctab_bytes = 0;
   struct Subtree {
      struct Key {
         long tips_gen = -1, tree_gen = -1, cherry_gen = -1, cap_mb = -1;
         double frac = -1;
         int K = -1;
         bool operator==(const Key &o) const { return tips_gen == o.tips_gen && tree_gen == o.tree_gen && cherry_gen == o.cherry_gen && cap_mb == o.cap_mb && frac == o.frac && K == o.K; }
      } made_for;
      long sel_gen = 0, zt_sel_gen = -1;
      int zt_tiles = 0, zt_tile_patt = 0;
      std::vector<unsigned int> u;
      std::vector<char> done;
      std::vector<std::vector<unsigned int>> cls, son_cls;
      std::vector<int> sel;
      SubtreeProgram sp;
      std::vector<int> level_first;
      std::vector<int> level_tiles;
      long rows = 0;
      long n_computed = 0;
      long n_order_computed = 0;
      bool ordered = false;
      std::vector<std::vector<unsigned int>> rowmap;
      std::vector<char> level_small;
      DevBuf<int> d_order;
      long order_sel_gen = -1;
      double order_host_s = 0;
      int zt_bytes = 0;
      DevBuf<SubtreeNodeDev> d_nodes;
      DevBuf<unsigned int> d_sidx, d_top_cls;
      DevBuf<int> d_meta;
      DevBuf<unsigned char> d_ztiles;
   } sub;
   std::vector<unsigned char> h_z;
   long tips_gen = 0, tree_gen = 0, cherry_gen = 0;
   DevBuf<double> d_stab;
   int n_stab = 0;
   bool stab_attr_set = false;
   long last_stab_n = 0, last_stab_bytes = 0, last_stab_blocks = -1;
   std::vector<JitKernel> jit_pool;
   std::vector<std::pair<std::string, int>> jit_seen;
   void jit_retire()
   {
      if (jit.mod && jit.fn) {
         if (jit_pool.size() >= 8) { (void)hipModuleUnload(jit_pool.front().mod); jit_pool.erase(jit_pool.begin()); }
         jit_pool.push_back(jit);
      }
      else if (jit.mod) (void)hipModuleUnload(jit.mod);
      jit = JitKernel();
   }
   bool jit_recall(const std::string &key)
   {
      if (jit.fn && jit.key == key) return true;
      for (size_t i = 0; i < jit_pool.size(); i++)
         if (jit_pool[i].key == key && jit_pool[i].fn) {
            const JitKernel k = jit_pool[i];
            jit_pool.erase(jit_pool.begin() + i);
            jit_retire();
            jit = k;
            return true;
         }
      return false;
   }
   int jit_count_request(const std::string &key)
   {
      for (auto &kv : jit_seen)
         if (kv.first == key) return ++kv.second;
      if (jit_seen.size() >= 64) jit_seen.erase(jit_seen.begin());
      jit_seen.emplace_back(key, 1);
      return 1;
   }
   bool jit_enabled = false;
   bool small20 = false;
   JitKernel jit_coop;
   bool coopj_enabled = true;
   bool pipe_ok = false;
   hipStream_t s2 = nullptr;
   hipEvent_t ev_entry[2] = {nullptr, nullptr}, ev_pmat = nullptr;
   int entry_sel = 0;
   bool have_prev_entry = false;
   static constexpr int NPSET = 6;
   struct PSet { DevBuf<double> rowmajor, pint, ptip, pcol, ctab, stab; int id = 0; } spare[NPSET - 1];
   int spare_head = 0;
   DevBuf<double> d2_branch, d2_gene_rate;
   hipStream_t sb[MAXL - 1] = {};
   hipEvent_t ev_setread[NPSET] = {};
   bool setread_rec[NPSET] = {};
   int pset = 0;
   bool dual_ok = false, dual_run = false;
   bool jit_forced = false;
   struct JitJob {
      std::thread th;
      std::atomic<int> state{0};
      std::string key, src, log;
      std::vector<char> code;
      JitJob() { worker_threads_list(&th, true); }
      ~JitJob() { if (th.joinable()) th.join(); worker_threads_list(&th, false); }
   };
   struct JitSlot {
      std::unique_ptr<JitJob> job;
      std::set<std::string> failed;
   };
   JitSlot jit_slot, coop_slot, bjit_slot;

   std::vector<EigenHost> eigen;
   std::vector<int> h_eigen_of;
   std::vector<double> h_qfactor;
   DevBuf<PmatRes> d_pres;
   bool pres_valid = false;
   int plain_codes = 0;
   bool amb_ascending = true;
   int pmat_B = 1;
   bool rowmajor_valid = false;
   DevBuf<EigenDev> d_eigen;
   DevBuf<double> d_eq_q, d_eq_pi, d_eq_scale;
   DevBuf<double *> d_eq_ptr;
   DevBuf<int> d_eq_rc;
// ... 3 lines not shown
   bool eigen_attr_set = false;
   bool eigen_warm = false;
   long n_eigen_warm = 0;
   long n_eigen_device = 0;
   int eq_last_batch = 0;
   bool eigen_dirty = true;

   int mode = PAML_AMD_MODE_LFUN, K = 1, n_labels = 1;

   DevBuf<double> d_b_qfactor, d_b_freqK, d_b_rate;
   DevBuf<double> d_beb_f, d_beb_part, d_beb_g, d_beb_out, d_beb_pcl;
   DevBuf<double> d_adg_all;
   DevBuf<int> d_beb_iw;
   DevBuf<double> d_rowmajor, d_pint, d_ptip, d_pcol, d_fhK, d_fscale, d_lnf, d_partial, d_out, d_partials, d_scalef, d_stack;
   DevBuf<double> d_expA, d_expB, d_expSA, d_expSB, d_deriv, d_tt, d_bpartial, d_bout;
   DevBuf<int> d_label_eff;
   DevBuf<Op> d_ops_tmp;
   bool partials_valid = false;

   bool profiling = false;
   std::vector<hipEvent_t> ev_pool;
   std::vector<hipEvent_t> ev_used;
   long prof_evals = 0;
   long n_eval = 0, n_pmat = 0;

   ~paml_amd_engine()
   {
      for (auto &e : eigen) { e.U.release(); e.V.release(); e.Root.release(); e.Cijk.release(); }
      stage.release();
      if (sc) (void)hipStreamSynchronize(sc);
      if (comm && rccl().CommDestroy) (void)rccl().CommDestroy(comm);
      if (sc) (void)hipStreamDestroy(sc);
      for (int b = 0; b < MAXL; b++) {
         if (ev_part[b]) (void)hipEventDestroy(ev_part[b]);
         if (ev_done[b]) (void)hipEventDestroy(ev_done[b]);
      }
      for (hipEvent_t ev : ev_bk)
         if (ev) (void)hipEventDestroy(ev);
      for (int i = 0; i < NSTAT; i++)
         for (hipEvent_t ev : {st_part[i], st_done[i], st_w0[i], st_w1[i]})
            if (ev) (void)hipEventDestroy(ev);
      if (h_out) (void)hipHostFree(h_out);
      if (h_eig_fail) (void)hipHostFree(h_eig_fail);
      for (int ln = 0; ln < MAXL && d_prof && env.prof_tiles && prof_words; ln++) {
         std::vector<unsigned long long> hp(prof_words);
         if (hipMemcpy(hp.data(), d_prof + (size_t)ln * prof_words, prof_words * 8, hipMemcpyDeviceToHost) == hipSuccess)
            if (FILE *f = fopen((env.prof_ops + (ln ? "." + std::to_string(ln) : std::string())).c_str(), "wb")) {
               const int hdr[2] = {prof_blocks, prof_stride};
               fwrite(hdr, sizeof(int), 2, f);
               std::vector<int> codes(prof_stride - 3, 0);
               fwrite(codes.data(), sizeof(int), codes.size(), f);
               fwrite(hp.data(), 8, hp.size(), f);
               fclose(f);
            }
      }
      if (d_prof) (void)hipFree(d_prof);
      if (jit.mod) (void)hipModuleUnload(jit.mod);
      for (JitKernel &k : jit_pool)
         if (k.mod) (void)hipModuleUnload(k.mod);
      if (jit_coop.mod) (void)hipModuleUnload(jit_coop.mod);
      for (auto ev : ev_pool) (void)hipEventDestroy(ev);
      for (auto ev : ev_used) (void)hipEventDestroy(ev);
      DevBuf<unsigned char> *b1[] = {&d_z, &d_chara_map, &d_is_leaf, &d_ztiles};
      for (auto b : b1) b->release();
      DevBuf<int> *b2[] = {&d_n_chara, &d_gene_off, &d_label, &d_eigen_of, &d_b_eigen_of, &d_beb_iw};
      for (auto b : b2) b->release();
      d_tiles.release();
      d_tiles_full.release();
      d_tile_group0.release();
      tile_stash.tiles.release(); tile_stash.group0.release(); tile_stash.ztip_of.release(); tile_stash.ztiles.release();
      d_ztip_of.release();
      d_zpm.release();
      d_red_counter.release();
      d_bl_partials.release(); d_bl_scalef.release(); d_bl_frag.release(); d_code_mask.release();
      d_bl_coef.release(); d_bl_efrag.release(); d_bl_ztab.release(); d_bl_etab.release(); d_bl_ecol.release();
      d_ops.release();
      d_ops_tmp.release();
      d_label_eff.release();
      d_stream.release();
      d_eigen.release();
      d_pres.release();
      d_ctab.release();
      d_stab.release();
      sub.d_nodes.release(); sub.d_sidx.release(); sub.d_top_cls.release(); sub.d_meta.release(); sub.d_ztiles.release(); sub.d_order.release();
      d_eq_q.release(); d_eq_pi.release(); d_eq_scale.release(); d_eq_ptr.release(); d_eq_rc.release(); d_eq_sweeps.release();
      d_pi_plain.release();
      DevBuf<double> *b3[] = {&d_weights, &d_pi, &d_freqK, &d_rate, &d_qfactor, &d_branch, &d_gene_rate, &d_rowmajor,
                              &d_pint, &d_ptip, &d_pcol, &d_fhK, &d_fscale, &d_lnf, &d_b_qfactor, &d_b_freqK, &d_b_rate, &d_beb_f, &d_beb_part, &d_beb_g, &d_beb_out, &d_beb_pcl, &d_adg_all, &d_partial, &d_out, &d_partials, &d_scalef, &d_stack, &d2_branch, &d2_gene_rate, &d_partial_tot, &d_btot,
                              &d_expA, &d_expB, &d_expSA, &d_expSB, &d_deriv, &d_tt, &d_bpartial, &d_bout};
      for (auto b : b3) b->release();
      for (auto &sp : spare) { sp.rowmajor.release(); sp.pint.release(); sp.ptip.release(); sp.pcol.release(); sp.ctab.release(); sp.stab.release(); }
      for (int b = 0; b < MAXL - 1; b++) { d_partial_s[b].release(); d_partial_tot_s[b].release(); d_fhK_s[b].release(); }
   }
};

namespace paml_amd {

inline int fail(paml_amd_engine *e, int code, const std::string &msg)
{
   if (e) e->err = msg;
   return code;
}

#define HIPCHK(call)                                                                                         \
   do {                                                                                                      \
      hipError_t _r = (call);                                                                                \
      if (_r != hipSuccess)                                                                                  \
         return fail(e, _r == hipErrorOutOfMemory ? PAML_AMD_ENOMEM : PAML_AMD_EHIP,                         \
                     std::string(#call) + ": " + hipGetErrorString(_r));                                     \
   } while (0)

template <typename T>
inline hipError_t upload(DevBuf<T> &b, const T *src, size_t n, hipStream_t s)
{
   hipError_t r = b.ensure(n);
   if (r != hipSuccess) return r;
   if (n == 0) return hipSuccess;
   return hipMemcpyAsync(b.p, src, n * sizeof(T), hipMemcpyHostToDevice, s);
}

inline int tipw(const paml_amd_engine *e) { return e->kk == KK_MFMA64 ? 64 : e->n; }
inline size_t tip_words(const paml_amd_engine *e)
{
   if (e->kk != KK_MFMA64) return (size_t)e->n_codes * e->n;
   return e->n_codes <= 64 ? 4096 : (size_t)e->n_codes * 64;
}
inline int pint_words(const paml_amd_engine *e) { return e->kk == KK_MFMA64 ? 4096 : e->n * e->n; }

inline std::vector<int> code_order(int n, int n_codes, const int *nch, const unsigned char *cmap, const long *cnt)
{
   std::vector<int> order(n_codes, -1), rest;
   std::vector<char> placed(n_codes, 0);
   for (int c = 0; c < n_codes; c++) {
      const int s = cmap[(size_t)c * n];
      if (nch[c] == 1 && s < n_codes && order[s] < 0) { order[s] = c; placed[c] = 1; }
   }
   for (int c = 0; c < n_codes; c++)
      if (!placed[c]) rest.push_back(c);
   std::stable_sort(rest.begin(), rest.end(), [&](int x, int y) { return cnt[x] * nch[x] > cnt[y] * nch[y]; });
   for (int i = 0, k = 0; i < n_codes; i++)
      if (order[i] < 0) order[i] = rest[k++];
   return order;
}

inline hipEvent_t get_event(paml_amd_engine *e)
{
   hipEvent_t ev;
   if (!e->ev_pool.empty()) {
      ev = e->ev_pool.back();
      e->ev_pool.pop_back();
   }
   else if (hipEventCreate(&ev) != hipSuccess)
      return nullptr;
   e->ev_used.push_back(ev);
   return ev;
}

inline void mark_on(paml_amd_engine *e, hipStream_t s)
{
   if (!e->profiling) return;
   hipEvent_t ev = get_event(e);
   if (ev) (void)hipEventRecord(ev, s);
}
inline void mark(paml_amd_engine *e) { mark_on(e, e->stream); }

inline hipError_t create_engine_stream(hipStream_t *s)
{
// ... 125 lines not shown
```

### paml_amd/csrc/kernels_prune.h

```cpp
#pragma once
#include <hip/hip_runtime.h>

#include "kernel_args.h"

namespace paml_amd {

#define MFMA_EPI_INTO(DST)                                                                                       \
   do {                                                                                                         \
      if (pop < 0) {                                                                                            \
         _Pragma("unroll") for (int m = 0; m < 16; m++) DST[m] = acc[m >> 2][m & 3];                            \
      }                                                                                                         \
      else if (pop == 0) {                                                                                      \
         _Pragma("unroll") for (int m = 0; m < 16; m++) DST[m] = s0[m] * acc[m >> 2][m & 3];                    \
      }                                                                                                         \
      else if (pop == 1) {                                                                                      \
         _Pragma("unroll") for (int m = 0; m < 16; m++) DST[m] = s1[m] * acc[m >> 2][m & 3];                    \
      }                                                                                                         \
      else {                                                                                                    \
         const double *sp2 = a.stack_scratch +                                                                  \
                             (((long)blockIdx.x * a.stack_overflow_slots + (pop - MFMA_RS)) * WAVES + wave) * 1024; \
         _Pragma("unroll") for (int m = 0; m < 16; m++) DST[m] = sp2[m * 64 + lane] * acc[m >> 2][m & 3];       \
      }                                                                                                         \
   } while (0)

#define MFMA_EPILOGUE()                                                                                          \
   do {                                                                                                         \
      const int pop = mm_pop_slot(op), push = mm_push_slot(op);                                                 \
      if (push < 0) MFMA_EPI_INTO(cur);                                                                         \
      else if (push == 0) MFMA_EPI_INTO(s0);                                                                    \
      else if (push == 1) MFMA_EPI_INTO(s1);                                                                    \
      else {                                                                                                    \
         double tmpv[16];                                                                                       \
         MFMA_EPI_INTO(tmpv);                                                                                   \
         double *sp3 = a.stack_scratch +                                                                        \
                       (((long)blockIdx.x * a.stack_overflow_slots + (push - MFMA_RS)) * WAVES + wave) * 1024;  \
         _Pragma("unroll") for (int m = 0; m < 16; m++) sp3[m * 64 + lane] = tmpv[m];                           \
      }                                                                                                         \
   } while (0)

#define MFMA_CORE_CASES()                                                                                        \
   case OP_INIT_ONES: {                                                                                         \
      _Pragma("unroll") for (int m = 0; m < 16; m++) cur[m] = (4 * m + q < n) ? 1.0 : 0.0;                      \
   } break;                                                                                                     \
   case OP_INIT_TIP: {                                                                                          \
      const int code = TIP_CODE(op.a);                                                                          \
      _Pragma("unroll") for (int m = 0; m < 16; m++) cur[m] = (a.cleandata && 4 * m + q == code) ? 1.0 : 0.0;   \
   } break;

#define MFMA_EXT_CASES()                                                                                         \
   case OP_PUSH: {                                                                                              \
      if (op.b == 0) { _Pragma("unroll") for (int m = 0; m < 16; m++) s0[m] = cur[m]; }                         \
      else if (op.b == 1) { _Pragma("unroll") for (int m = 0; m < 16; m++) s1[m] = cur[m]; }                    \
      else {                                                                                                    \
         double *sp = a.stack_scratch +                                                                         \
                      (((long)blockIdx.x * a.stack_overflow_slots + (op.b - MFMA_RS)) * WAVES + wave) * 1024;   \
         _Pragma("unroll") for (int m = 0; m < 16; m++) sp[m * 64 + lane] = cur[m];                             \
      }                                                                                                         \
   } break;                                                                                                     \
   case OP_SCALE: {                                                                                             \
      double mx = 0;                                                                                            \
      _Pragma("unroll") for (int m = 0; m < 16; m++) mx = cur[m] > mx ? cur[m] : mx;                            \
      double o = __shfl_xor(mx, 16);                                                                            \
      mx = o > mx ? o : mx;                                                                                     \
      o = __shfl_xor(mx, 32);                                                                                   \
      mx = o > mx ? o : mx;                                                                                     \
      double fac;                                                                                               \
      if (mx < 1e-300) {                                                                                        \
         _Pragma("unroll") for (int m = 0; m < 16; m++) cur[m] = (4 * m + q < n) ? 1.0 : 0.0;                   \
         fac = -800;                                                                                            \
      }                                                                                                         \
      else {                                                                                                    \
         _Pragma("unroll") for (int m = 0; m < 16; m++) cur[m] /= mx;                                           \
         fac = log(mx);                                                                                         \
      }                                                                                                         \
      lnscale += fac;                                                                                           \
      if (a.keep && q == 0 && valid) a.scalef[((long)iclass * a.n_scale + op.b) * a.n_patt + h] = fac;          \
   } break;                                                                                                     \
   case OP_STORE: {   \
      double *dst = a.partials + (((long)iclass * a.n_int + (op.a - a.n_tips)) * (long)a.part_groups +          \
                                  ((long)tile * WAVES + wave)) * 1024;                                          \
      part_store(dst, lane, cur);                                                                               \
   } break;                                                                                                     \
   case OP_LOAD: {                                                                                              \
      const double *src = a.partials + (((long)iclass * a.n_int + (op.a - a.n_tips)) * (long)a.part_groups +    \
                                        ((long)tile * WAVES + wave)) * 1024;                                    \
// ... 579 lines not shown
         }
         lnscale += fac;
         if (a.keep && valid) a.scalef[((long)iclass * a.n_scale + op.b) * a.n_patt + h] = fac;
      } break;
      case OP_STORE: {
         if (valid) {
            double *dst = a.partials + (((long)iclass * a.n_int + (op.a - a.n_tips)) * a.n_patt + h) * N;
#pragma unroll
            for (int j = 0; j < N; j++) dst[j] = cur[j];
         }
      } break;
      case OP_LOAD: {
         const double *src = a.partials + (((long)iclass * a.n_int + (op.a - a.n_tips)) * a.n_patt + hc) * N;
#pragma unroll
         for (int j = 0; j < N; j++) cur[j] = src[j];
      } break;
      case OP_EXPORT: {
         if (valid) {
            double *dst = a.export_buf + ((long)iclass * a.n_patt + h) * N;
#pragma unroll
            for (int j = 0; j < N; j++) dst[j] = cur[j];
            if (a.export_scale) a.export_scale[(long)iclass * a.n_patt + h] = lnscale;
         }
      } break;
      case OP_ROOT: {
         const double *pi = a.pi + (long)(a.n_pi > 1 ? gene : 0) * N;
         double f = 0;
#pragma unroll
         for (int j = 0; j < N; j++) f = fma(pi[j], cur[j], f);
         if (a.keep && a.n_scale) {
            lnscale = 0;
            if (valid)
               for (int k = 0; k < a.n_scale; k++) lnscale += a.scalef[((long)iclass * a.n_scale + k) * a.n_patt + h];
         }
         if (valid) {
            double out = 0;
            if (a.weights[h] > 0) out = root_value(a, f, lnscale);
            a.fhK[(long)iclass * a.n_patt + h] = out;
         }
      } break;
      default: break;
      }
   }
}

__global__ __launch_bounds__(256) void ztile_kernel(const int2 *tiles, const int *gene_off, const unsigned char *z, long z_stride,
                                                    const double *weights, int n_tips, int zt_bytes, unsigned char *out, const int *tip_of, const int *row_at)
{
   const int t = blockIdx.x, i = threadIdx.x, tp = blockDim.x;
   const int g = tiles[t].x, h = tiles[t].y + i, hend = gene_off[g + 1];
   unsigned char *o = out + (long)t * zt_bytes;
   for (int k = i; k < zt_bytes; k += tp) o[k] = 0;
   __syncthreads();
   for (int r = 0; r <= n_tips; r++) {
      const int tip = tip_of ? tip_of[r] : r;
      const long at = (long)(tip_of ? row_at[r] : r) * tp;
      unsigned char v = 0;
      if (h < hend) v = tip < n_tips ? z[tip * z_stride + h] : (unsigned char)(weights[h] > 0 ? 1 : 0);
      o[at + i] = v;
   }
}

__global__ __launch_bounds__(256) void sztile_kernel(const int2 *tiles, const int *gene_off, const unsigned char *z, long z_stride, const double *weights,
                                                     int n_tips, int zt_bytes, unsigned char *out, int n_top, const unsigned int *top_cls, const int *order)
{
   const int t = blockIdx.x, i = threadIdx.x, tp = blockDim.x;
   const int g = tiles[t].x, pos = tiles[t].y + i, hend = gene_off[g + 1];
   const bool in = pos < hend;
   const int h = in ? (order ? order[pos] : pos) : 0;
   unsigned char *o = out + (long)t * zt_bytes;
   for (int k = i; k < zt_bytes; k += tp) o[k] = 0;
   __syncthreads();
   for (int r = 0; r <= n_tips; r++) {
      unsigned char v = 0;
      if (in) v = r < n_tips ? z[r * z_stride + h] : (unsigned char)(weights[h] > 0 ? 1 : 0);
      o[(long)r * tp + i] = v;
   }
   for (int k = 0; k < n_top; k++) {
      const unsigned int c = in ? top_cls[(long)k * z_stride + h] : 0u;
      for (int b = 0; b < 3; b++) o[(long)(n_tips + 1 + 3 * k + b) * tp + i] = (unsigned char)((c >> (8 * b)) & 255u);
   }
}

__global__ __launch_bounds__(256) void zpm_kernel(const unsigned char *z, long z_stride, int n_tips, int n_patt, int zw, unsigned int *out)
{
   const long h = (long)blockIdx.x * 256 + threadIdx.x;
   if (h >= n_patt) return;
   for (int w = 0; w < zw; w++) {
      unsigned int v = 0;
      for (int b = 0; b < 4; b++) {
         const int t = 4 * w + b;
         if (t < n_tips) v |= (unsigned int)z[t * z_stride + h] << (8 * b);
      }
      out[h * zw + w] = v;
   }
}

}
```

### paml_amd/engine.py

```python
from __future__ import annotations

import ctypes as C
import os
import subprocess

import numpy as np

from .problem import EIGEN_CIJK, EIGEN_JC69LIKE, EIGEN_K80, EIGEN_QMAT, EIGEN_UVROOT, Problem

_HERE = os.path.dirname(os.path.abspath(__file__))
LIB_PATH = os.environ.get("PAML_AMD_LIB") or os.path.join(_HERE, "lib", "libpaml_amd.so")
CSRC = os.path.join(_HERE, "csrc")
KEEP_PARTIALS = 1
JIT = 2
SHARD = 4

EXPORTS = [
    "paml_amd_set_gene_class_rates", "paml_amd_get_branch_partials", "paml_amd_create", "paml_amd_destroy", "paml_amd_last_error", "paml_amd_set_stream", "paml_amd_set_tips",
    "paml_amd_set_tree", "paml_amd_set_pi", "paml_amd_set_eigen_uvroot", "paml_amd_set_eigen_cijk",
    "paml_amd_set_eigen_qrev_batch", "paml_amd_set_eigen_qrev_batch_sparse", "paml_amd_set_eigen_warm_start", "paml_amd_get_eigen", "paml_amd_eigen_counters", "paml_amd_set_eigen_k80", "paml_amd_set_eigen_jc69like", "paml_amd_set_eigen_qmat", "paml_amd_set_classes", "paml_amd_eval",
    "paml_amd_eval_batch", "paml_amd_eval_adg", "paml_amd_beb_grid", "paml_amd_beb_grid_classes", "paml_amd_compress_patterns", "paml_amd_eval_device", "paml_amd_eval_dirty", "paml_amd_eval_branch", "paml_amd_node_posterior", "paml_amd_get_pmat", "paml_amd_get_partials", "paml_amd_get_scale",
    "paml_amd_device_count", "paml_amd_set_device", "paml_amd_shard_bounds", "paml_amd_max_ranks", "paml_amd_flush", "paml_amd_eigen_status", "paml_amd_comm_unique_id", "paml_amd_comm_init", "paml_amd_comm_destroy", "paml_amd_comm_info", "paml_amd_comm_library", "paml_amd_comm_stats", "paml_amd_get_partial_sums", "paml_amd_branch_counters", "paml_amd_branch_coef_hits", "paml_amd_branch_refill_kernels", "paml_amd_branch_kernel_ms",
    "paml_amd_jit_prebuild", "paml_amd_profile", "paml_amd_profile_read", "paml_amd_counters", "paml_amd_kernel_name", "paml_amd_debug_program", "paml_amd_debug_jit",
    "paml_amd_cherry_tables", "paml_amd_debug_jit_tables",
    "paml_amd_subtree_tables", "paml_amd_subtree_order", "paml_amd_debug_subtree_order", "paml_amd_debug_subtree_classes", "paml_amd_debug_jit_subtree", "paml_amd_debug_subtree_select",
    "paml_amd_debug_code_order", "paml_amd_debug_branch_plan",
    "paml_amd_pairset_create", "paml_amd_pairset_destroy", "paml_amd_pairset_get_counts", "paml_amd_pairset_set_pi", "paml_amd_pairset_set_pattern",
    "paml_amd_pairset_eval", "paml_amd_pairset_failed", "paml_amd_pairset_counters",
    "paml_amd_rell_replicates", "paml_amd_rell_info",
    "paml_amd_simulate", "paml_amd_simulate_info",
    "paml_amd_ancestral_marginal", "paml_amd_ancestral_joint", "paml_amd_ancestral_info",
    "paml_amd_gradient", "paml_amd_gradient_info",
    "paml_amd_model_gradient", "paml_amd_model_gradient_info", "paml_amd_model_gradient_segment", "paml_amd_model_gradient_sizes",
    "paml_amd_nni_scores", "paml_amd_nni_info", "paml_amd_nni_list",
    "paml_amd_edge_scores", "paml_amd_edge_info", "paml_amd_edge_list",
    "paml_amd_placement_scores", "paml_amd_placement_info",
    "paml_amd_spr_scores", "paml_amd_spr_info", "paml_amd_spr_list",
]


class EngineError(RuntimeError):
    pass


UNIT_FLAGS = {}
EXTRA_FLAGS = os.environ.get("PAML_AMD_EXTRA_FLAGS", "").split()
UNITS = ("engine_core", "engine_comm", "engine_eval", "engine_branch", "engine_beb", "engine_jitdbg", "engine_compress", "engine_pairwise", "engine_rell", "engine_simulate", "engine_ancestral", "engine_gradient", "engine_modelgrad", "engine_nni", "engine_place", "engine_spr", "engine_edge")


def build(force: bool = False, verbose: bool = False) -> str:
    import glob
    from concurrent.futures import ThreadPoolExecutor
    hdrs = glob.glob(os.path.join(CSRC, "*.h")) + [os.path.join(os.path.dirname(_HERE), "include", "paml_amd.h")]
    newest_hdr = max(os.path.getmtime(h) for h in hdrs)
    hipcc = os.environ.get("HIPCC", "/opt/rocm/bin/hipcc")
    objdir = os.path.join(os.path.dirname(LIB_PATH), "obj")
    os.makedirs(objdir, exist_ok=True)
    jobs = []
    for u in UNITS:
        src, obj = os.path.join(CSRC, u + ".hip"), os.path.join(objdir, u + ".o")
        if force or not os.path.exists(obj) or os.path.getmtime(obj) < max(newest_hdr, os.path.getmtime(src)):
            jobs.append([hipcc, "--offload-arch=gfx950", "-O3", "-std=c++17", "-fPIC"] + UNIT_FLAGS.get(u, []) + EXTRA_FLAGS + ["-c", src, "-o", obj])
    objs = [os.path.join(objdir, u + ".o") for u in UNITS]
    if not jobs and os.path.exists(LIB_PATH) and all(os.path.getmtime(o) <= os.path.getmtime(LIB_PATH) for o in objs):
        return LIB_PATH

    def run(cmd):
        if verbose:
            print(" ".join(cmd), flush=True)
        subprocess.check_call(cmd)
    with ThreadPoolExecutor(max_workers=max(1, min(len(jobs), os.cpu_count() or 1))) as ex:
        list(ex.map(run, jobs))
    run([hipcc, "--offload-arch=gfx950", "-shared", "-fPIC", "-o", LIB_PATH] + objs + ["-lhiprtc", "-ldl"])
    return LIB_PATH


_LIB = None


def lib():
    global _LIB
    if _LIB is None:
        if not os.path.exists(LIB_PATH):
            raise EngineError("libpaml_amd.so is not built (run python -c 'import __graft_entry__ as g; g.build()')")
        L = C.CDLL(LIB_PATH)
        L.paml_amd_last_error.restype = C.c_char_p
        L.paml_amd_kernel_name.restype = C.c_char_p
        L.paml_amd_destroy.restype = None
        L.paml_amd_create.argtypes = [C.POINTER(C.c_void_p), C.c_int, C.c_int, C.c_int, C.c_int, C.c_int, C.c_uint]
        L.paml_amd_destroy.argtypes = [C.c_void_p]
        L.paml_amd_last_error.argtypes = [C.c_void_p]
        L.paml_amd_kernel_name.argtypes = [C.c_void_p]
        L.paml_amd_set_stream.argtypes = [C.c_void_p, C.c_void_p]
        L.paml_amd_set_tips.argtypes = [C.c_void_p, C.c_void_p, C.c_int, C.c_int, C.c_void_p, C.c_void_p, C.c_void_p, C.c_void_p]
        L.paml_amd_set_tree.argtypes = [C.c_void_p, C.c_int, C.c_int, C.c_void_p, C.c_void_p, C.c_void_p, C.c_void_p]
        L.paml_amd_set_pi.argtypes = [C.c_void_p, C.c_int, C.c_void_p]
        L.paml_amd_set_eigen_uvroot.argtypes = [C.c_void_p, C.c_int, C.c_void_p, C.c_void_p, C.c_void_p]
        L.paml_amd_set_eigen_cijk.argtypes = [C.c_void_p, C.c_int, C.c_int, C.c_void_p, C.c_void_p]
        L.paml_amd_set_eigen_qrev_batch.argtypes = [C.c_void_p, C.c_int, C.c_void_p, C.c_void_p, C.c_void_p, C.c_void_p]
        L.paml_amd_set_eigen_qrev_batch_sparse.argtypes = [C.c_void_p, C.c_int, C.c_void_p, C.c_int, C.c_void_p, C.c_void_p, C.c_void_p, C.c_void_p, C.c_void_p]
        L.paml_amd_get_eigen.argtypes = [C.c_void_p, C.c_int, C.c_void_p, C.c_void_p, C.c_void_p]
        L.paml_amd_eigen_counters.argtypes = [C.c_void_p, C.POINTER(C.c_long), C.c_void_p, C.c_int]
        L.paml_amd_set_eigen_k80.argtypes = [C.c_void_p, C.c_int, C.c_double]
        L.paml_amd_set_eigen_jc69like.argtypes = [C.c_void_p, C.c_int]
        L.paml_amd_set_classes.argtypes = [C.c_void_p, C.c_int, C.c_int, C.c_void_p, C.c_void_p, C.c_int, C.c_void_p, C.c_void_p]
        L.paml_amd_eval.argtypes = [C.c_void_p, C.c_void_p, C.c_void_p, C.POINTER(C.c_double), C.c_void_p, C.c_void_p]
        L.paml_amd_eval_device.argtypes = [C.c_void_p, C.c_void_p, C.c_void_p, C.c_void_p]
        L.paml_amd_eval_dirty.argtypes = [C.c_void_p, C.c_void_p, C.c_void_p, C.c_void_p, C.POINTER(C.c_double)]
# ... 397 lines not shown

    def placement_scores(self, branch, gene_rate=None, queries=None, edges=None, pendant=(0.1,), phi=0.5, pendant_label=0, want_lnf=False):
        b = np.ascontiguousarray(branch, dtype=np.float64)
        g = None if gene_rate is None else np.ascontiguousarray(gene_rate, dtype=np.float64)
        if queries is None:
            raise EngineError("placement_scores: no queries")
        qz = np.ascontiguousarray(np.atleast_2d(queries), dtype=np.uint8)
        if qz.ndim != 2 or qz.shape[1] != self.n_patt:
            raise EngineError("placement_scores: queries must be [n_q][n_patt]")
        if edges is None:
            if getattr(self, "_tree_csr", None) is None:
                raise EngineError("placement_scores: no tree was set through this object")
            edges = [v for v in range(self.n_nodes) if v != self._tree_csr[0]]
        ed = np.ascontiguousarray(edges, dtype=np.int32).reshape(-1)
        pe = np.ascontiguousarray(np.atleast_1d(pendant), dtype=np.float64).reshape(-1)
        lnL0 = C.c_double()
        lnL = np.zeros((len(qz), len(ed), len(pe)))
        lnf = np.zeros((len(qz), len(ed), len(pe), self.n_patt)) if want_lnf else None
        self._L.paml_amd_placement_scores.argtypes = [C.c_void_p, C.c_void_p, C.c_void_p, C.c_int, C.c_void_p, C.c_int, C.c_void_p, C.c_int, C.c_void_p,
                                                      C.c_double, C.c_int, C.POINTER(C.c_double), C.c_void_p, C.c_void_p]
        self._chk(self._L.paml_amd_placement_scores(self._h, _p(b), _p(g), len(qz), _p(qz), len(ed), _p(ed), len(pe), _p(pe), float(phi),
                                                    int(pendant_label), C.byref(lnL0), _p(lnL), _p(lnf)))
        return dict(lnL0=lnL0.value, edges=ed, lnL=lnL, lnf=lnf)

    def spr_scores(self, branch, gene_rate=None, moves=None, radius=0, phi=0.5, want_lnf=False):
        b = np.ascontiguousarray(branch, dtype=np.float64)
        g = None if gene_rate is None else np.ascontiguousarray(gene_rate, dtype=np.float64)
        if moves is None:
            if getattr(self, "_tree_csr", None) is None:
                raise EngineError("spr_scores: no tree was set through this object")
            moves = spr_list(self.n_tips, self.n_nodes, *self._tree_csr, radius=radius)
        mv = np.ascontiguousarray(moves, dtype=np.int32).reshape(-1, 2)
        lnL0 = C.c_double()
        lnL = np.zeros(len(mv))
        lnf = np.zeros((len(mv), self.n_patt)) if want_lnf else None
        self._L.paml_amd_spr_scores.argtypes = [C.c_void_p, C.c_void_p, C.c_void_p, C.c_int, C.c_void_p, C.c_double, C.POINTER(C.c_double), C.c_void_p, C.c_void_p]
        self._chk(self._L.paml_amd_spr_scores(self._h, _p(b), _p(g), len(mv), _p(mv), float(phi), C.byref(lnL0), _p(lnL), _p(lnf)))
        return dict(lnL0=lnL0.value, moves=mv, lnL=lnL, lnf=lnf)

    def get_pmat(self, gene, iclass, node):
        P = np.zeros((self.n, self.n))
        self._chk(self._L.paml_amd_get_pmat(self._h, gene, iclass, node, _p(P)))
        return P

    def get_partials(self, node, iclass=0):
        a = np.zeros((self.n_patt, self.n))
        self._chk(self._L.paml_amd_get_partials(self._h, node, iclass, _p(a)))
        return a

    def get_scale(self, node, iclass=0):
        a = np.zeros(self.n_patt)
        self._chk(self._L.paml_amd_get_scale(self._h, node, iclass, _p(a)))
        return a

    def profile(self, on=True):
        self._chk(self._L.paml_amd_profile(self._h, int(on)))

    def profile_read(self):
        a, b, c, n = C.c_double(), C.c_double(), C.c_double(), C.c_long()
        self._chk(self._L.paml_amd_profile_read(self._h, C.byref(a), C.byref(b), C.byref(c), C.byref(n)))
        return dict(ms_pmat=a.value, ms_prune=b.value, ms_reduce=c.value, n_evals=n.value)

    def cherry_tables(self):
        a, b = C.c_long(), C.c_long()
        self._L.paml_amd_cherry_tables.argtypes = [C.c_void_p, C.POINTER(C.c_long), C.POINTER(C.c_long)]
        self._chk(self._L.paml_amd_cherry_tables(self._h, C.byref(a), C.byref(b)))
        return a.value, b.value

    def subtree_tables(self):
        cap = 256
        n, by, bl, nc = C.c_long(), C.c_long(), C.c_long(), C.c_long()
        nodes, u = np.zeros(cap, dtype=np.int32), np.zeros(cap, dtype=np.int64)
        self._L.paml_amd_subtree_tables.argtypes = [C.c_void_p, C.POINTER(C.c_long), C.c_void_p, C.c_void_p, C.c_int] + [C.POINTER(C.c_long)] * 3
        self._chk(self._L.paml_amd_subtree_tables(self._h, C.byref(n), _p(nodes), _p(u), cap, C.byref(by), C.byref(bl), C.byref(nc)))
        k = min(n.value, cap)
        return dict(nodes=nodes[:k].tolist(), u=u[:k].tolist(), bytes=by.value, blocks_left=bl.value, n_computed=nc.value)

    def subtree_order(self):
        use, nc, sec = C.c_int(), C.c_long(), C.c_double()
        self._L.paml_amd_subtree_order.argtypes = [C.c_void_p, C.POINTER(C.c_int), C.POINTER(C.c_long), C.POINTER(C.c_double)]
        self._chk(self._L.paml_amd_subtree_order(self._h, C.byref(use), C.byref(nc), C.byref(sec)))
        return dict(in_use=bool(use.value), n_computed=nc.value, host_seconds=sec.value)

    def counters(self):
        a, b = C.c_long(), C.c_long()
        self._L.paml_amd_counters(self._h, C.byref(a), C.byref(b))
        return dict(n_eval=a.value, n_pmat=b.value)


class PairSet:

    def __init__(self, eng: Engine, pairs):
        pr = np.ascontiguousarray(pairs, dtype=np.int32).reshape(-1, 2)
        a, b = np.ascontiguousarray(pr[:, 0]), np.ascontiguousarray(pr[:, 1])
        L = eng._L
        L.paml_amd_pairset_create.argtypes = [C.c_void_p, C.POINTER(C.c_void_p), C.c_int, C.c_void_p, C.c_void_p]
        L.paml_amd_pairset_destroy.argtypes = [C.c_void_p]
        L.paml_amd_pairset_destroy.restype = None
        L.paml_amd_pairset_get_counts.argtypes = [C.c_void_p, C.c_void_p, C.c_void_p]
        L.paml_amd_pairset_set_pi.argtypes = [C.c_void_p, C.c_void_p]
        L.paml_amd_pairset_set_pattern.argtypes = [C.c_void_p, C.c_int, C.c_void_p, C.c_void_p, C.c_void_p]
        L.paml_amd_pairset_eval.argtypes = [C.c_void_p, C.c_long] + [C.c_void_p] * 5
        L.paml_amd_pairset_failed.argtypes = [C.c_void_p, C.c_void_p, C.c_long]
        L.paml_amd_pairset_counters.argtypes = [C.c_void_p] + [C.POINTER(C.c_long)] * 4
        self._eng, self._L, self.n, self.n_pairs = eng, L, eng.n, len(pr)
        h = C.c_void_p()
        eng._chk(L.paml_amd_pairset_create(eng._h, C.byref(h), len(pr), _p(a), _p(b)))
        self._h = h

    def close(self):
        if getattr(self, "_h", None):
            self._L.paml_amd_pairset_destroy(self._h)
            self._h = None

    def __del__(self):
        try:
            self.close()
        except Exception:
            pass

    def counts(self):
        fp, ls = np.zeros((self.n_pairs, self.n, self.n)), np.zeros(self.n_pairs)
        self._eng._chk(self._L.paml_amd_pairset_get_counts(self._h, _p(fp), _p(ls)))
        return fp, ls

    def set_pi(self, pi):
        pi = np.ascontiguousarray(pi, dtype=np.float64)
        assert pi.shape == (self.n_pairs, self.n)
        self._eng._chk(self._L.paml_amd_pairset_set_pi(self._h, _p(pi)))

    def set_pattern(self, row, col, flags):
        row, col = np.ascontiguousarray(row, dtype=np.int32), np.ascontiguousarray(col, dtype=np.int32)
        fl = np.ascontiguousarray(flags, dtype=np.uint8)
        assert len(row) == len(col) == len(fl)
        self._eng._chk(self._L.paml_amd_pairset_set_pattern(self._h, len(row), _p(row), _p(col), _p(fl)))

    def eval(self, pair, t, kappa, omega):
        pr = np.ascontiguousarray(pair, dtype=np.int32)
        t, k, w = (np.ascontiguousarray(np.broadcast_to(np.asarray(x, dtype=np.float64), pr.shape)) for x in (t, kappa, omega))
        out = np.zeros(len(pr))
        self._eng._chk(self._L.paml_amd_pairset_eval(self._h, len(pr), _p(pr), _p(t), _p(k), _p(w), _p(out)))
        return out

    def failed(self):
        n = self._L.paml_amd_pairset_failed(self._h, None, 0)
        idx = np.zeros(max(n, 1), dtype=np.int64)
        self._L.paml_amd_pairset_failed(self._h, _p(idx), n)
        return idx[:n]

    def counters(self):
        v = [C.c_long() for _ in range(4)]
        self._L.paml_amd_pairset_counters(self._h, *[C.byref(x) for x in v])
        return dict(n_elem=v[0].value, n_decomp=v[1].value, n_chunks=v[2].value, arena_slots=v[3].value)


COMM_ID_BYTES = 128


def shard_bounds(n_patt_global, world, rank):
    first, count = C.c_long(), C.c_long()
    rc = lib().paml_amd_shard_bounds(int(n_patt_global), int(world), int(rank), C.byref(first), C.byref(count))
    if rc != 0:
        raise EngineError("paml_amd_shard_bounds(%d patterns, world %d) failed (%d): at most %d ranks for this many patterns"
                          % (n_patt_global, world, rc, lib().paml_amd_max_ranks(int(n_patt_global))))
    return first.value, count.value

# ... 54 lines not shown
    ops = np.zeros((cap, 4), dtype=np.int32)
    L.paml_amd_debug_branch_plan.argtypes = [C.c_int, C.c_int, C.c_int, C.c_void_p, C.c_void_p, C.c_void_p, C.c_int, C.c_void_p, C.c_void_p,
                                             C.c_void_p, C.c_void_p, C.c_void_p, C.c_void_p, C.c_int]
    nops = L.paml_amd_debug_branch_plan(tree.n_tips, tree.n_nodes, tree.root, _p(ptr), _p(flat), _p(sc), len(calls), _p(nb), _p(br),
                                        _p(ends), _p(up), _p(clean), _p(ops), cap)
    if nops < 0:
        raise EngineError("debug_branch_plan failed (%d)" % nops)
    return ends, up, clean, [tuple(int(v) for v in r) for r in ops[:nops]]


def debug_code_order(n_states, n_chara, chara_map, z):
    L = lib()
    nch = np.ascontiguousarray(n_chara, dtype=np.int32)
    cm = np.ascontiguousarray(chara_map, dtype=np.uint8)
    zz = np.ascontiguousarray(z, dtype=np.uint8).ravel()
    order = np.zeros(len(nch), dtype=np.int32)
    L.paml_amd_debug_code_order.argtypes = [C.c_int, C.c_int, C.c_void_p, C.c_void_p, C.c_void_p, C.c_long, C.c_void_p]
    rc = L.paml_amd_debug_code_order(int(n_states), len(nch), _p(nch), _p(cm), _p(zz), zz.size, _p(order))
    if rc < 0:
        raise EngineError("debug_code_order failed (%d)" % rc)
    return order


def debug_jit(tree, scale_node=None, compile=True, n_states=0, fused=None):
    L = lib()
    ptr, flat = tree.csr()
    sc = None if scale_node is None else np.ascontiguousarray(scale_node, dtype=np.uint8)
    cap = 1 << 20
    buf = C.create_string_buffer(cap)
    L.paml_amd_debug_jit.argtypes = [C.c_int, C.c_int, C.c_int, C.c_void_p, C.c_void_p, C.c_void_p, C.c_char_p, C.c_int, C.c_int]
    flags = int(bool(compile)) | (int(n_states) << 8)
    if fused:
        flags |= 2 | (int(fused[0]) << 16) | (int(fused[1]) << 24) | ((int(fused[2]) // 256 if len(fused) > 2 else 1) << 2)
    rc = L.paml_amd_debug_jit(tree.n_tips, tree.n_nodes, tree.root, _p(ptr), _p(flat), _p(sc), buf, cap, flags)
    if rc < 0:
        raise EngineError("debug_jit failed (%d): %s" % (rc, buf.value.decode(errors="replace")[-3000:]))
    return buf.value.decode()


def debug_jit_tables(tree, scale_node=None, max_tabs=1 << 20):
    L = lib()
    ptr, flat = tree.csr()
    sc = None if scale_node is None else np.ascontiguousarray(scale_node, dtype=np.uint8)
    cap = 1 << 21
    buf = C.create_string_buffer(cap)
    stream = np.zeros(4 * tree.n_nodes + 8, dtype=np.int32)
    tabs = np.zeros(3 * tree.n_tips + 3, dtype=np.int32)
    ns = C.c_int()
    L.paml_amd_debug_jit_tables.argtypes = [C.c_int, C.c_int, C.c_int, C.c_void_p, C.c_void_p, C.c_void_p, C.c_int, C.c_char_p, C.c_int,
                                            C.c_void_p, C.c_int, C.POINTER(C.c_int), C.c_void_p, C.c_int]
    rc = L.paml_amd_debug_jit_tables(tree.n_tips, tree.n_nodes, tree.root, _p(ptr), _p(flat), _p(sc), int(max_tabs), buf, cap,
                                     _p(stream), len(stream), C.byref(ns), _p(tabs), len(tabs))
    if rc < 0:
        raise EngineError("debug_jit_tables failed (%d)" % rc)
    return buf.value.decode(), [tuple(x) for x in stream[:2 * ns.value].reshape(-1, 2)], [tuple(x) for x in tabs[:3 * rc].reshape(-1, 3)]


def debug_subtree_classes(tree, z, n_codes, want_classes=False):
    L = lib()
    ptr, flat = tree.csr()
    z = np.ascontiguousarray(z, dtype=np.uint8)
    n_patt = z.shape[1]
    u = np.zeros(tree.n_nodes, dtype=np.uint32)
    cls = np.zeros((tree.n_nodes, n_patt), dtype=np.uint32) if want_classes else None
    L.paml_amd_debug_subtree_classes.argtypes = [C.c_int, C.c_int, C.c_int, C.c_void_p, C.c_void_p, C.c_void_p, C.c_long, C.c_int, C.c_void_p, C.c_void_p]
    rc = L.paml_amd_debug_subtree_classes(tree.n_tips, tree.n_nodes, tree.root, _p(ptr), _p(flat), _p(z), n_patt, int(n_codes), _p(u), _p(cls))
    if rc < 0:
        raise EngineError("debug_subtree_classes failed (%d)" % rc)
    return (u, cls) if want_classes else u


def debug_subtree_order(keys, bound, largest_first=False, as_given=False):
    L = lib()
    keys = np.ascontiguousarray(keys, dtype=np.uint32)
    bound = np.ascontiguousarray(bound, dtype=np.uint32)
    out = np.zeros(keys.shape[1], dtype=np.uint32)
    L.paml_amd_debug_subtree_order.argtypes = [C.c_int, C.c_void_p, C.c_void_p, C.c_long, C.c_int, C.c_int, C.c_void_p]
    rc = L.paml_amd_debug_subtree_order(keys.shape[0], _p(keys), _p(bound), keys.shape[1], int(largest_first), int(as_given), _p(out))
    if rc < 0:
        raise EngineError("debug_subtree_order failed (%d)" % rc)
    return out


def debug_subtree_select(tree, z, n_states, n_codes, K=1, scale_node=None):
    L = lib()
    ptr, flat = tree.csr()
    z = np.ascontiguousarray(z, dtype=np.uint8)
    sc = None if scale_node is None else np.ascontiguousarray(scale_node, dtype=np.uint8)
    sel = np.zeros(tree.n_nodes, dtype=np.int32)
    L.paml_amd_debug_subtree_select.argtypes = [C.c_int, C.c_int, C.c_int, C.c_void_p, C.c_void_p, C.c_void_p, C.c_int, C.c_int, C.c_int, C.c_void_p, C.c_long,
                                                C.c_void_p, C.c_int]
    n = L.paml_amd_debug_subtree_select(tree.n_tips, tree.n_nodes, tree.root, _p(ptr), _p(flat), _p(sc), int(n_states), int(n_codes), int(K), _p(z), z.shape[1],
                                        _p(sel), len(sel))
    if n < 0:
        raise EngineError("debug_subtree_select failed (%d)" % n)
    return sel[:n].tolist()


def debug_jit_subtree(tree, nodes, n_states=61, n_codes=61, K=1, compile=True, scale_node=None, directory=None):
    L = lib()
    ptr, flat = tree.csr()
    sc = None if scale_node is None else np.ascontiguousarray(scale_node, dtype=np.uint8)
    sel = np.ascontiguousarray(nodes, dtype=np.int32)
    cap = 1 << 21
    buf = C.create_string_buffer(cap)
    left = C.c_int(-1)
    L.paml_amd_debug_jit_subtree.argtypes = [C.c_int, C.c_int, C.c_int, C.c_void_p, C.c_void_p, C.c_void_p, C.c_int, C.c_int, C.c_int, C.c_void_p, C.c_int,
                                             C.c_int, C.c_char_p, C.c_char_p, C.c_int, C.POINTER(C.c_int)]
    if directory:
        os.makedirs(directory, exist_ok=True)
    rc = L.paml_amd_debug_jit_subtree(tree.n_tips, tree.n_nodes, tree.root, _p(ptr), _p(flat), _p(sc), int(n_states), int(n_codes), int(K), _p(sel), len(sel),
                                      int(bool(compile)), os.fsencode(directory) if directory else None, buf, cap, C.byref(left))
    if rc < 0:
        raise EngineError("debug_jit_subtree failed (%d): %s" % (rc, buf.value.decode(errors="replace")[-3000:]))
    if rc == 0:
        return "", None
    return buf.value.decode(), left.value


JIT_SHIPPED_DIR = os.path.join(_HERE, "lib", "jit")


def jit_prebuild(tree, n_states, n_codes, K=1, n_patt_global=1_000_000, scale_node=None, directory=None):
    L = lib()
    ptr, flat = tree.csr()
    sc = None if scale_node is None else np.ascontiguousarray(scale_node, dtype=np.uint8)
    d = directory or JIT_SHIPPED_DIR
    os.makedirs(d, exist_ok=True)
    log = C.create_string_buffer(1 << 16)
    L.paml_amd_jit_prebuild.argtypes = [C.c_int, C.c_int, C.c_int, C.c_int, C.c_long, C.c_int, C.c_int, C.c_void_p, C.c_void_p, C.c_void_p,
                                        C.c_char_p, C.c_char_p, C.c_int]
    rc = L.paml_amd_jit_prebuild(int(n_states), tree.n_tips, int(n_codes), int(K), int(n_patt_global), tree.n_nodes, tree.root, _p(ptr), _p(flat),
                                 _p(sc), os.fsencode(d), log, len(log))
    if rc != 0:
        raise EngineError("jit_prebuild failed (%d): %s" % (rc, log.value.decode(errors="replace")[-2000:]))


def compress_patterns(chars, gene=None):
    chars = np.ascontiguousarray(chars, dtype=np.uint8)
    width = 1 if chars.ndim == 2 else chars.shape[2]
    n_seq, n_sites = chars.shape[0], chars.shape[1]
    g = None if gene is None else np.ascontiguousarray(gene, dtype=np.int32)
    npatt = C.c_int()
    first, w, pose = np.zeros(n_sites, dtype=np.int32), np.zeros(n_sites), np.zeros(n_sites, dtype=np.int32)
    L = lib()
    L.paml_amd_compress_patterns.argtypes = [C.c_int, C.c_int, C.c_int, C.c_void_p, C.c_void_p, C.POINTER(C.c_int), C.c_void_p, C.c_void_p, C.c_void_p]
    rc = L.paml_amd_compress_patterns(n_seq, n_sites, width, _p(chars), _p(g), C.byref(npatt), _p(first), _p(w), _p(pose))
    if rc != 0:
        raise EngineError("paml_amd_compress_patterns failed (%d)" % rc)
    return dict(first_site=first[:npatt.value].copy(), weights=w[:npatt.value].copy(), pose=pose)


def rell_info():
    v, ms = [C.c_int() for _ in range(3)], C.c_double()
    L = lib()
    L.paml_amd_rell_info.argtypes = [C.POINTER(C.c_int)] * 3 + [C.POINTER(C.c_double)]
    L.paml_amd_rell_info.restype = None
    L.paml_amd_rell_info(*[C.byref(x) for x in v], C.byref(ms))
    return dict(chunk=v[0].value, tree_block=v[1].value, last_batches=v[2].value, last_kernel_ms=ms.value)


def simulate_info():
    L = lib()
    nb, ms = C.c_int(), C.c_double()
    L.paml_amd_simulate_info.argtypes = [C.POINTER(C.c_int), C.POINTER(C.c_double)]
    L.paml_amd_simulate_info.restype = None
# ... 138 lines not shown
```

Before: 4.535 billion site-patterns/s.

## Add gather-walk kernel that prunes via deduplicated table-row lookups per tile

When the per-tree program reduces to a chain of cherry/subtree table lookups followed by the root, a host planner groups ordered patterns into tiles of up to 128 with at most R distinct table rows. It packs per-tile descriptors, and a new kernel DMAs the deduplicated rows into LDS with double-buffered descriptor and row prefetch, then multiplies the rows and does the root reduction. This replaces the JIT MFMA kernel path with an LDS-gather walk that is meant to cut redundant global reads of table rows. The cost is host-side tile planning and extra LDS use, and the path applies only when the program shape qualifies.

```diff
diff --git a/include/paml_amd.h b/include/paml_amd.h
--- a/include/paml_amd.h
+++ b/include/paml_amd.h
@@ -116,6 +116,7 @@
 int paml_amd_cherry_tables(const paml_amd_engine *e, long *n_tabulated, long *bytes);
 int paml_amd_subtree_tables(const paml_amd_engine *e, long *n_tabulated, int *nodes, long *u, int cap, long *bytes, long *blocks_left, long *n_computed);
 int paml_amd_subtree_order(const paml_amd_engine *e, int *in_use, long *n_computed, double *host_seconds);
+int paml_amd_gather_walk(const paml_amd_engine *e, int *in_use, long *n_tiles, long *n_rows, int *R, long *n_computed, double *host_seconds);
 
 int paml_amd_debug_program(int n_tips, int n_nodes, int root, const int *sons_ptr, const int *sons,
                            const unsigned char *scale_node, int keep_partials, const unsigned char *clean,
@@ -140,6 +141,9 @@
 
 int paml_amd_debug_subtree_order(int n_keys, const unsigned int *keys, const unsigned int *bound, long n_patt, int largest_first, int as_given,
                                  unsigned int *order_out);
+
+int paml_amd_debug_gather_tiles(int n_keys, const unsigned int *keys, const unsigned int *bound, const unsigned int *order, const unsigned char *wflag,
+                                long n_patt, int R, unsigned char *blocks_out, long cap_bytes, long *n_tiles, long *n_rows);
 
 int paml_amd_debug_subtree_select(int n_tips, int n_nodes, int root, const int *sons_ptr, const int *sons, const unsigned char *scale_node, int n_states,
                                   int n_codes, int K, const unsigned char *z, long n_patt, int *sel_out, int cap);
diff --git a/paml_amd/csrc/device_common.h b/paml_amd/csrc/device_common.h
--- a/paml_amd/csrc/device_common.h
+++ b/paml_amd/csrc/device_common.h
@@ -77,6 +77,9 @@
    long stab_rows;
    const int *stab_meta;
    const int *order;
+   const unsigned char *gw_desc;
+   int gw_tiles, gw_desc_bytes, gw_R;
+   int gw_kind[4], gw_id[4];
 };
 
 __device__ __forceinline__ double root_value(const PruneArgs &a, double f, double lnscale)
diff --git a/paml_amd/csrc/engine_core.hip b/paml_amd/csrc/engine_core.hip
--- a/paml_amd/csrc/engine_core.hip
+++ b/paml_amd/csrc/engine_core.hip
@@ -183,8 +183,12 @@
    for (int g = 0; g < e->n_genes; g++)
       if (e->gene_off[g + 1] < e->gene_off[g]) return fail(e, PAML_AMD_EINVAL, "set_tips: gene_off must not decrease");
    HIPCHK(upload(e->d_z, z, nz, e->stream));
-   if (e->kk == KK_MFMA64 && e->n_genes == 1 && n_codes <= 64) e->h_z.assign(z, z + nz);
-   else std::vector<unsigned char>().swap(e->h_z);
+   if (e->kk == KK_MFMA64 && e->n_genes == 1 && n_codes <= 64) {
+      e->h_z.assign(z, z + nz);
+      e->h_wflag.resize(e->n_patt);
+      for (long h = 0; h < e->n_patt; h++) e->h_wflag[h] = weights[h] > 0 ? 1 : 0;
+   }
+   else { std::vector<unsigned char>().swap(e->h_z); std::vector<unsigned char>().swap(e->h_wflag); }
    e->tips_gen++;
    HIPCHK(upload(e->d_weights, weights, (size_t)e->n_patt, e->stream));
    HIPCHK(upload(e->d_n_chara, nch.data(), nch.size(), e->stream));
@@ -753,6 +757,18 @@
    return 0;
 }
 
+int paml_amd_gather_walk(const paml_amd_engine *e, int *in_use, long *n_tiles, long *n_rows, int *R, long *n_computed, double *host_seconds)
+{
+   if (!e) return PAML_AMD_EINVAL;
+   if (in_use) *in_use = (e->last_stab_n && e->last_gw) ? 1 : 0;
+   if (n_tiles) *n_tiles = e->sub.gw_tiles;
+   if (n_rows) *n_rows = e->sub.gw_rows;
+   if (R) *R = e->sub.gw_R;
+   if (n_computed) *n_computed = e->sub.gw_computed;
+   if (host_seconds) *host_seconds = e->sub.gw_host_s;
+   return 0;
+}
+
 int paml_amd_counters(const paml_amd_engine *e, long *n_eval, long *n_pmat)
 {
    if (!e) return PAML_AMD_EINVAL;
diff --git a/paml_amd/csrc/engine_eval.hip b/paml_amd/csrc/engine_eval.hip
--- a/paml_amd/csrc/engine_eval.hip
+++ b/paml_amd/csrc/engine_eval.hip
@@ -445,6 +445,7 @@
       sb.order_host_s = std::chrono::duration<double>(std::chrono::steady_clock::now() - t0).count();
       HIPCHK(upload(sb.d_order, (const int *)order.data(), order.size(), e->stream));
       HIPCHK(hipStreamSynchronize(e->stream));
+      sb.h_order = order;
       sb.order_sel_gen = sb.sel_gen;
       sb.n_order_computed++;
    }
@@ -456,6 +457,87 @@
    HIPCHK(hipStreamSynchronize(e->stream));
    sb.d_top_cls.release();
    sb.zt_sel_gen = sb.sel_gen; sb.zt_tiles = e->n_tiles; sb.zt_tile_patt = e->tile_patt;
+   return 0;
+}
+
+static bool gather_walk_wanted()
+{
+   const char *v = getenv("PAML_AMD_GATHER_WALK");
+   return !v || atoi(v) != 0;
+}
+static void gather_walk_plan(paml_amd_engine *e)
+{
+   paml_amd_engine::Subtree &sb = e->sub;
+   if (sb.gw_plan_gen == sb.sel_gen) return;
+   sb.gw_plan_gen = sb.sel_gen;
+   sb.gw_ok = false;
+   sb.gw_nlk = 0;
+   const Program &p = sb.sp.prog;
+   if (!p.stream.empty() || e->tree.n_scale || e->n_pi != 1 || e->n_genes != 1 || e->h_wflag.size() != (size_t)e->n_patt) return;
+   bool have_cur = false, rooted = false;
+   int n = 0, slot = -1;
+   for (const Op &o : p.ops) {
+      if (o.code == OP_END) break;
+      if (o.code == OP_ROOT) {
+         if (!have_cur || rooted) return;
+         rooted = true;
+         continue;
+      }
+      if (o.code != OP_LOOKUP || rooted || have_cur || n == GATHER_MAX_LOOKUPS) return;
+      const int pop = mm_pop_slot(o), push = mm_push_slot(o);
+      if (n == 0 ? (pop >= 0 || push < 0) : (pop != slot || (push >= 0 && push != slot))) return;
+      if (n == 0) slot = push;
+      have_cur = push < 0;
+      const bool sub = o.c >= SUBTREE_TAB_BASE;
+      const long rows = sub ? (long)sb.u[sb.sp.sub[sb.sp.top[o.c - SUBTREE_TAB_BASE]].node] : (long)e->n_codes * e->n_codes;
+      if (rows < 1 || rows * (long)CHERRY_ROW_BYTES >= (1L << 31)) return;
+      sb.gw_kind[n] = sub ? 0 : 1; sb.gw_id[n] = sub ? o.c - SUBTREE_TAB_BASE : o.c;
+      n++;
+   }
+   if (!rooted || n < 2) return;
+   sb.gw_nlk = n;
+   sb.gw_ok = true;
+}
+
+int ensure_gather_tiles(paml_amd_engine *e)
+{
+   paml_amd_engine::Subtree &sb = e->sub;
+   gather_walk_plan(e);
+   if (!sb.gw_ok) return 0;
+   const int R = e->env.gather_R;
+   if (sb.gw_sel_gen == sb.sel_gen && sb.gw_R == R && sb.gw_ordered == sb.ordered) return 0;
+   if (sb.d_gw_desc.p) HIPCHK(hipDeviceSynchronize());
+   const auto t0 = std::chrono::steady_clock::now();
+   const long np = e->n_patt;
+   std::vector<std::vector<unsigned int>> cls(sb.gw_nlk, std::vector<unsigned int>(np));
+   std::vector<const unsigned int *> keys;
+   std::vector<unsigned int> bound;
+   for (int k = 0; k < sb.gw_nlk; k++) {
+      if (sb.gw_kind[k] == 0) {
+         const int ti = sb.sp.top[sb.gw_id[k]];
+         const std::vector<unsigned int> &c = sb.cls[sb.sp.sub[ti].node], &rm = sb.rowmap[ti];
+         const unsigned int u = sb.u[sb.sp.sub[ti].node];
+         for (long h = 0; h < np; h++) cls[k][h] = std::min(rm.empty() ? c[h] : rm[c[h]], u - 1);
+         bound.push_back(u);
+      }
+      else {
+         const CherryTab &ct = sb.sp.tabs[sb.gw_id[k]];
+         const unsigned char *za = e->h_z.data() + (size_t)ct.tip_a * np, *zb = e->h_z.data() + (size_t)ct.tip_b * np;
+         const unsigned int nc = (unsigned int)e->n_codes;
+         for (long h = 0; h < np; h++) cls[k][h] = std::min((unsigned int)za[h], nc - 1) * nc + std::min((unsigned int)zb[h], nc - 1);
+         bound.push_back(nc * nc);
+      }
+      keys.push_back(cls[k].data());
+   }
+   const bool ordered = sb.ordered && sb.h_order.size() == (size_t)np;
+   const unsigned int *order = ordered ? sb.h_order.data() : nullptr;
+   const GatherTiles g = gather_tiles(keys, bound, order, np, R);
+   const std::vector<unsigned char> blocks = gather_tiles_pack(g, order, e->h_wflag.data(), np);
+   sb.gw_host_s = std::chrono::duration<double>(std::chrono::steady_clock::now() - t0).count();
+   HIPCHK(upload(sb.d_gw_desc, blocks.data(), blocks.size(), e->stream));
+   HIPCHK(hipStreamSynchronize(e->stream));
+   sb.gw_tiles = (long)g.n_tiles(); sb.gw_rows = g.total_rows(); sb.gw_R = R; sb.gw_sel_gen = sb.sel_gen; sb.gw_ordered = sb.ordered;
+   sb.gw_computed++;
    return 0;
 }
 
@@ -522,6 +604,8 @@
       if (int r = select_tiles(e, big_tiles, want_waves, jit_ok)) return r;
       if (e->n_stab)
          if (int r = ensure_subtree_ztiles(e)) return r;
+      if (e->n_stab && jit_ok && gather_walk_wanted() && e->env.prof_ops.empty() && !e->env.prof_tiles)
+         if (int r = ensure_gather_tiles(e)) return r;
       if (jit_ok || e->mfma_dma) {
          *out = jit_ok ? PK_MFMA64_JIT : PK_MFMA64_STREAM;
          return 0;
@@ -757,6 +841,14 @@
       pr.ztiles = e->sub.d_ztiles.p; pr.zt_bytes = e->sub.zt_bytes;
       pr.order = e->sub.ordered ? e->sub.d_order.p : nullptr;
    }
+   const paml_amd_engine::Subtree &gsb = e->sub;
+   const bool gather = k == PK_MFMA64_JIT && e->n_stab && !bs && gather_walk_wanted() && e->env.prof_ops.empty() && !e->env.prof_tiles && gsb.gw_ok &&
+                       gsb.gw_sel_gen == gsb.sel_gen && gsb.gw_ordered == gsb.ordered && gsb.gw_tiles > 0 && gsb.d_gw_desc.p;
+   e->last_gw = gather;
+   if (gather) {
+      pr.gw_desc = gsb.d_gw_desc.p; pr.gw_tiles = (int)gsb.gw_tiles; pr.gw_desc_bytes = gather_desc_bytes(gsb.gw_R); pr.gw_R = gsb.gw_R;
+      for (int i = 0; i < 4; i++) { pr.gw_kind[i] = gsb.gw_kind[i]; pr.gw_id[i] = gsb.gw_id[i]; }
+   }
    const int nb = (e->n_patt + e->chunk - 1) / e->chunk;
    if (pk_forms_reduction(k)) {
       pr.Km = c.Km; pr.chunk = e->chunk; pr.first_chunk = e->first_chunk; pr.nb_stride = e->nb_global;
@@ -788,6 +880,20 @@
    hipStream_t const ms = c.ms;
    switch (k) {
    case PK_MFMA64_JIT:
+      if (gather) {
+         const size_t lds = gather_walk_lds_bytes(pr.gw_R);
+         if (!e->gw_attr_set) {
+            HIPCHK(hipFuncSetAttribute((const void *)gather_walk_kernel<2>, hipFuncAttributeMaxDynamicSharedMemorySize, (int)gather_walk_lds_bytes(128)));
+            HIPCHK(hipFuncSetAttribute((const void *)gather_walk_kernel<3>, hipFuncAttributeMaxDynamicSharedMemorySize, (int)gather_walk_lds_bytes(128)));
+            HIPCHK(hipFuncSetAttribute((const void *)gather_walk_kernel<4>, hipFuncAttributeMaxDynamicSharedMemorySize, (int)gather_walk_lds_bytes(128)));
+            e->gw_attr_set = true;
+         }
+         const dim3 gg(std::min(pr.gw_tiles * K, cus)), gb(512);
+         if (gsb.gw_nlk == 2) hipLaunchKernelGGL(gather_walk_kernel<2>, gg, gb, lds, ms, pr);
+         else if (gsb.gw_nlk == 3) hipLaunchKernelGGL(gather_walk_kernel<3>, gg, gb, lds, ms, pr);
+         else hipLaunchKernelGGL(gather_walk_kernel<4>, gg, gb, lds, ms, pr);
+         break;
+      }
       HIPCHK(hipModuleLaunchKernel(e->jit.fn, std::min(n_blocks, cus), 1, 1, e->mfma_waves * 64, 1, 1, 0, ms, params, nullptr));
       break;
    case PK_MFMA64_STREAM:
diff --git a/paml_amd/csrc/engine_jitdbg.hip b/paml_amd/csrc/engine_jitdbg.hip
--- a/paml_amd/csrc/engine_jitdbg.hip
+++ b/paml_amd/csrc/engine_jitdbg.hip
@@ -199,6 +199,31 @@
    return 0;
 }
 
+int paml_amd_debug_gather_tiles(int n_keys, const unsigned int *keys, const unsigned int *bound, const unsigned int *order, const unsigned char *wflag,
+                                long n_patt, int R, unsigned char *blocks_out, long cap_bytes, long *n_tiles, long *n_rows)
+{
+   if (n_keys < 1 || n_keys > GATHER_MAX_LOOKUPS || n_patt < 1 || !keys || !bound || R < n_keys || R > GATHER_R_MAX) return PAML_AMD_EINVAL;
+   std::vector<const unsigned int *> k(n_keys);
+   std::vector<unsigned int> b(bound, bound + n_keys);
+   for (int i = 0; i < n_keys; i++) k[i] = keys + (long)i * n_patt;
+   for (long i = 0; i < (long)n_keys * n_patt; i++)
+      if (keys[i] >= bound[i / n_patt]) return PAML_AMD_EINVAL;
+   if (order) {
+      std::vector<char> seen(n_patt, 0);
+      for (long i = 0; i < n_patt; i++) {
+         if (order[i] >= (unsigned long)n_patt || seen[order[i]]) return PAML_AMD_EINVAL;
+         seen[order[i]] = 1;
+      }
+   }
+   const GatherTiles g = gather_tiles(k, b, order, n_patt, R);
+   const std::vector<unsigned char> ones(wflag ? 0 : n_patt, 1);
+   const std::vector<unsigned char> blocks = gather_tiles_pack(g, order, wflag ? wflag : ones.data(), n_patt);
+   if (n_tiles) *n_tiles = (long)g.n_tiles();
+   if (n_rows) *n_rows = g.total_rows();
+   if (blocks_out) memcpy(blocks_out, blocks.data(), std::min((size_t)std::max(0L, cap_bytes), blocks.size()));
+   return gather_desc_bytes(R);
+}
+
 int paml_amd_debug_subtree_select(int n_tips, int n_nodes, int root, const int *sons_ptr, const int *sons, const unsigned char *scale_node, int n_states,
                                   int n_codes, int K, const unsigned char *z, long n_patt, int *sel_out, int cap)
 {
diff --git a/paml_amd/csrc/engine_state.h b/paml_amd/csrc/engine_state.h
--- a/paml_amd/csrc/engine_state.h
+++ b/paml_amd/csrc/engine_state.h
@@ -26,6 +26,7 @@
 #include "program.h"
 #include "branch_plan.h"
 #include "subtree_classes.h"
+#include "gather_tiles.h"
 
 namespace paml_amd {
 static_assert(JIT_SCRATCH_BASE == MFMA_RS, "the per-tree kernel addresses the interpreter's overflow-stack scratch");
@@ -170,6 +171,7 @@
    double subtree_max_frac = 0.5;
    long subtree_cap_mb = 2048;
    int subtree_order = 1;
+   int gather_R = 128;
    int subtree_rows = 1;
    std::string jit_dump, prof_ops;
    int prof_tid = 0;
@@ -196,6 +198,7 @@
       if (const char *v = getenv("PAML_AMD_SUBTREE_CAP_MB")) subtree_cap_mb = std::max(0L, atol(v));
       if (const char *v = getenv("PAML_AMD_SUBTREE_ORDER")) subtree_order = std::max(0, std::min(2, atoi(v)));
       if (const char *v = getenv("PAML_AMD_SUBTREE_ROWS")) subtree_rows = atoi(v) != 0 ? 1 : 0;
+      if (const char *v = getenv("PAML_AMD_GATHER_R")) gather_R = std::max(8, std::min(128, atoi(v))) & ~1;
       if (const char *v = getenv("PAML_AMD_JIT_DUMP")) jit_dump = v;
       if (const char *v = getenv("PAML_AMD_PROF_OPS")) prof_ops = v;
       if (const char *v = getenv("PAML_AMD_PROF_TID")) prof_tid = atoi(v);
@@ -364,8 +367,15 @@
       DevBuf<unsigned int> d_sidx, d_top_cls;
       DevBuf<int> d_meta;
       DevBuf<unsigned char> d_ztiles;
+      std::vector<unsigned int> h_order;
+      DevBuf<unsigned char> d_gw_desc;
+      long gw_sel_gen = -1, gw_plan_gen = -1, gw_tiles = 0, gw_rows = 0, gw_computed = 0;
+      int gw_R = 0, gw_nlk = 0, gw_kind[4] = {0, 0, 0, 0}, gw_id[4] = {0, 0, 0, 0};
+      bool gw_ok = false, gw_ordered = false;
+      double gw_host_s = 0;
    } sub;
-   std::vector<unsigned char> h_z;
+   bool gw_attr_set = false, last_gw = false;
+   std::vector<unsigned char> h_z, h_wflag;
    long tips_gen = 0, tree_gen = 0, cherry_gen = 0;
    DevBuf<double> d_stab;
    int n_stab = 0;
@@ -535,7 +545,7 @@
       d_pres.release();
       d_ctab.release();
       d_stab.release();
-      sub.d_nodes.release(); sub.d_sidx.release(); sub.d_top_cls.release(); sub.d_meta.release(); sub.d_ztiles.release(); sub.d_order.release();
+      sub.d_nodes.release(); sub.d_sidx.release(); sub.d_top_cls.release(); sub.d_meta.release(); sub.d_ztiles.release(); sub.d_order.release(); sub.d_gw_desc.release();
       d_eq_q.release(); d_eq_pi.release(); d_eq_scale.release(); d_eq_ptr.release(); d_eq_rc.release(); d_eq_sweeps.release();
       d_pi_plain.release();
       DevBuf<double> *b3[] = {&d_weights, &d_pi, &d_freqK, &d_rate, &d_qfactor, &d_branch, &d_gene_rate, &d_rowmajor,
diff --git a/paml_amd/csrc/gather_tiles.h b/paml_amd/csrc/gather_tiles.h
--- /dev/null
+++ b/paml_amd/csrc/gather_tiles.h
@@ -0,0 +1,110 @@
+#pragma once
+#include <cstdint>
+#include <cstring>
+#include <vector>
+
+namespace paml_amd {
+
+constexpr int GATHER_TILE_PATT = 128;
+constexpr int GATHER_MAX_LOOKUPS = 4;
+constexpr int GATHER_R_MAX = 160;
+
+struct GatherTiles {
+   int n_lookups = 0, R = 0;
+   std::vector<uint32_t> first, count;
+   std::vector<uint32_t> list_at;
+   std::vector<uint32_t> rows;
+   std::vector<uint8_t> slot;
+   size_t n_tiles() const { return first.size(); }
+   long total_rows() const { return (long)rows.size(); }
+};
+
+inline GatherTiles gather_tiles(const std::vector<const uint32_t *> &cls, const std::vector<uint32_t> &bound, const uint32_t *order, long n_patt, int R)
+{
+   GatherTiles g;
+   g.n_lookups = (int)cls.size();
+   g.R = R;
+   const int nk = g.n_lookups;
+   if (n_patt <= 0 || nk < 1 || R < nk) return g;
+   g.slot.assign((size_t)nk * n_patt, 0);
+   std::vector<std::vector<uint32_t>> seen_in(nk);
+   std::vector<std::vector<uint8_t>> slot_of(nk);
+   for (int k = 0; k < nk; k++) { seen_in[k].assign(bound[k], 0); slot_of[k].assign(bound[k], 0); }
+   std::vector<std::vector<uint32_t>> open(nk);
+   uint32_t tile_first = 0, tile_count = 0;
+   int distinct = 0;
+   auto close = [&]() {
+      g.first.push_back(tile_first);
+      g.count.push_back(tile_count);
+      for (int k = 0; k < nk; k++) {
+         g.list_at.push_back((uint32_t)g.rows.size());
+         g.rows.insert(g.rows.end(), open[k].begin(), open[k].end());
+         open[k].clear();
+      }
+      distinct = 0;
+      tile_count = 0;
+   };
+   for (long pos = 0; pos < n_patt; pos++) {
+      const long h = order ? (long)order[pos] : pos;
+      const uint32_t tile_id = (uint32_t)g.first.size() + 1;
+      int fresh = 0;
+      for (int k = 0; k < nk; k++) fresh += seen_in[k][cls[k][h]] != tile_id;
+      if (tile_count && (tile_count == (uint32_t)GATHER_TILE_PATT || distinct + fresh > R)) close();
+      if (!tile_count) tile_first = (uint32_t)pos;
+      const uint32_t id = (uint32_t)g.first.size() + 1;
+      for (int k = 0; k < nk; k++) {
+         const uint32_t r = cls[k][h];
+         if (seen_in[k][r] != id) {
+            seen_in[k][r] = id;
+            slot_of[k][r] = (uint8_t)open[k].size();
+            open[k].push_back(r);
+            distinct++;
+         }
+         g.slot[(size_t)k * n_patt + pos] = slot_of[k][r];
+      }
+      tile_count++;
+   }
+   if (tile_count) close();
+   g.list_at.push_back((uint32_t)g.rows.size());
+   return g;
+}
+
+constexpr int gather_desc_slots(int R) { return R + GATHER_MAX_LOOKUPS; }
+constexpr int gather_desc_off_slot(int R) { return 32 + 4 * gather_desc_slots(R); }
+constexpr int gather_desc_off_flag(int R) { return gather_desc_off_slot(R) + GATHER_MAX_LOOKUPS * GATHER_TILE_PATT; }
+constexpr int gather_desc_off_patt(int R) { return gather_desc_off_flag(R) + GATHER_TILE_PATT; }
+constexpr int gather_desc_bytes(int R) { return (gather_desc_off_patt(R) + 4 * GATHER_TILE_PATT + 255) / 256 * 256; }
+
+inline std::vector<unsigned char> gather_tiles_pack(const GatherTiles &g, const uint32_t *order, const unsigned char *wflag, long n_patt)
+{
+   const int R = g.R, nk = g.n_lookups, DB = gather_desc_bytes(R);
+   std::vector<unsigned char> out(g.n_tiles() * (size_t)DB, 0);
+   for (size_t t = 0; t < g.n_tiles(); t++) {
+      unsigned char *d = out.data() + t * (size_t)DB;
+      int32_t head[8] = {(int32_t)g.first[t], (int32_t)g.count[t], 0, 0, 0, 0, 0, 0};
+      uint32_t *rows = (uint32_t *)(d + 32);
+      int at = 0, start[GATHER_MAX_LOOKUPS] = {0, 0, 0, 0};
+      for (int k = 0; k < nk; k++) {
+         start[k] = at;
+         const uint32_t b = g.list_at[t * nk + k], e = g.list_at[t * nk + k + 1];
+         for (uint32_t i = b; i < e; i++) rows[at++] = g.rows[i];
+         if (at & 1) { rows[at] = rows[at - 1]; at++; }
+      }
+      for (int k = nk; k < GATHER_MAX_LOOKUPS; k++) start[k] = at;
+      head[2] = start[1]; head[3] = start[2]; head[4] = start[3]; head[5] = at;
+      memcpy(d, head, sizeof head);
+      unsigned char *slot = d + gather_desc_off_slot(R), *flag = d + gather_desc_off_flag(R);
+      int32_t *patt = (int32_t *)(d + gather_desc_off_patt(R));
+      const long h_first = order ? (long)order[g.first[t]] : (long)g.first[t];
+      for (int i = 0; i < GATHER_TILE_PATT; i++) {
+         const bool in = (uint32_t)i < g.count[t];
+         const long pos = (long)g.first[t] + i, h = in ? (order ? (long)order[pos] : pos) : h_first;
+         for (int k = 0; k < nk; k++) slot[k * GATHER_TILE_PATT + i] = (unsigned char)(start[k] + (in ? g.slot[(size_t)k * n_patt + pos] : 0));
+         flag[i] = in && wflag[h] ? 1 : 0;
+         patt[i] = (int32_t)h;
+      }
+   }
+   return out;
+}
+
+}
diff --git a/paml_amd/csrc/kernels_prune.h b/paml_amd/csrc/kernels_prune.h
--- a/paml_amd/csrc/kernels_prune.h
+++ b/paml_amd/csrc/kernels_prune.h
@@ -1,6 +1,7 @@
 #pragma once
 #include <hip/hip_runtime.h>
 
+#include "gather_tiles.h"
 #include "kernel_args.h"
 
 namespace paml_amd {
@@ -746,6 +747,109 @@
    }
 }
 
+constexpr int GW_PIECE_BYTES = 1024 + 64;
+constexpr int GW_DESC_BUFS = 3;
+constexpr size_t gather_walk_lds_bytes(int R) { return (size_t)2 * (gather_desc_slots(R) / 2) * GW_PIECE_BYTES + (size_t)GW_DESC_BUFS * gather_desc_bytes(R) + 64 * sizeof(double); }
+
+__device__ __forceinline__ void gw_dma16(__amdgpu_buffer_rsrc_t r, const void *lds, int voff)
+{
+   const unsigned la = __builtin_amdgcn_readfirstlane((unsigned)(unsigned long long)(__attribute__((address_space(3))) const char *)lds);
+   asm volatile("s_mov_b32 m0, %0\n\ts_nop 0\n\tbuffer_load_dwordx4 %1, %2, 0 offen lds" : : "s"(la), "v"(voff), "s"(r) : "memory", "m0");
+}
+
+template <int NLK>
+__global__ __launch_bounds__(512, 4) void gather_walk_kernel(PruneArgs a)
+{
+   extern __shared__ __attribute__((aligned(16))) unsigned char gw_smem[];
+   const int R = a.gw_R, DB = a.gw_desc_bytes, RB = (gather_desc_slots(R) / 2) * GW_PIECE_BYTES;
+   unsigned char *const rowbuf = gw_smem;
+   unsigned char *const descbuf = gw_smem + 2 * RB;
+   double *const sPi = (double *)(descbuf + GW_DESC_BUFS * DB);
+   const int tid = threadIdx.x, lane = tid & 63;
+   const int wave = __builtin_amdgcn_readfirstlane(tid >> 6);
+   const int q = lane >> 4, hl = lane & 15, p = wave * 16 + hl;
+   const int total = a.gw_tiles * a.K, step = gridDim.x;
+   if ((int)blockIdx.x >= total) return;
+   if (tid < 64) sPi[tid] = a.pi[tid];
+   const int nc2 = a.n_codes * a.n_codes;
+
+   auto issue_desc = [&](int work, int d) {
+      const int tile = work % a.gw_tiles;
+      if (wave * 256 < DB) dma4(make_rsrc(a.gw_desc + (long)tile * DB, DB), descbuf + d * DB + wave * 256, lane * 4, wave * 256);
+   };
+   auto issue_rows = [&](int work, int d, int b) {
+      const int iclass = work / a.gw_tiles;
+      const int *head = (const int *)(descbuf + d * DB);
+      const unsigned int *rows = (const unsigned int *)(descbuf + d * DB + 32);
+      const int s1 = __builtin_amdgcn_readfirstlane(head[2]), s2 = __builtin_amdgcn_readfirstlane(head[3]), s3 = __builtin_amdgcn_readfirstlane(head[4]);
+      int ns = __builtin_amdgcn_readfirstlane(head[5]);
+      ns = ns < gather_desc_slots(R) ? ns : (gather_desc_slots(R) & ~1);
+      const double *tab[NLK];
+      unsigned int bytes[NLK];
+#pragma unroll
+      for (int k = 0; k < NLK; k++) {
+         if (a.gw_kind[k]) { tab[k] = a.ctab + ((long)iclass * a.n_ctab + a.gw_id[k]) * (long)nc2 * CHERRY_ROW_WORDS; bytes[k] = (unsigned int)nc2 * 512u; }
+         else { tab[k] = JIT_STAB(iclass, a.gw_id[k]); bytes[k] = (unsigned int)JIT_STAB_U(a.gw_id[k]) * 512u; }
+      }
+      for (int j = wave; 2 * j < ns; j += 8) {
+         const int k = (2 * j >= s1) + (2 * j >= s2) + (2 * j >= s3);
+         const double *t = tab[0];
+         unsigned int nb = bytes[0];
+#pragma unroll
+         for (int kk = 1; kk < NLK; kk++)
+            if (k == kk) { t = tab[kk]; nb = bytes[kk]; }
+         const unsigned int row = rows[2 * j + (lane >> 5)];
+         gw_dma16(make_rsrc(t, nb), rowbuf + b * RB + j * GW_PIECE_BYTES, (int)(row * 512u + (unsigned int)((lane & 31) ^ ((lane >> 5) << 1)) * 16u));
+      }
+   };
+   auto landed = [&]() {
+      asm volatile("s_waitcnt vmcnt(0)" ::: "memory");
+      __syncthreads();
+   };
+
+   int work = blockIdx.x;
+   issue_desc(work, 0);
+   landed();
+   issue_rows(work, 0, 0);
+   if (work + step < total) issue_desc(work + step, 1);
+   landed();
+   for (int t = 0; work < total; work += step, t++) {
+      const int d = t % GW_DESC_BUFS, b = t & 1;
+      if (work + step < total) issue_rows(work + step, (t + 1) % GW_DESC_BUFS, b ^ 1);
+      if (work + 2 * step < total) issue_desc(work + 2 * step, (t + 2) % GW_DESC_BUFS);
+      {
+         const int iclass = work / a.gw_tiles;
+         const unsigned char *D = descbuf + d * DB;
+         const int np = ((const int *)D)[1];
+         const bool valid = p < np;
+         const unsigned char *rb = rowbuf + b * RB;
+         auto row_of = [&](int k, v4d (&x)[4]) {
+            const int s = D[gather_desc_off_slot(R) + k * GATHER_TILE_PATT + p];
+            const unsigned char *r = rb + (s >> 1) * GW_PIECE_BYTES + (s & 1) * 512 + (q ^ ((s & 1) << 1)) * 16;
+#pragma unroll
+            for (int i = 0; i < 8; i++) {
+               const part2_t v = *(const part2_t *)(r + i * 64);
+               x[i >> 1][(2 * i) & 3] = v.x;
+               x[i >> 1][(2 * i + 1) & 3] = v.y;
+            }
+         };
+         const int flag = D[gather_desc_off_flag(R) + p];
+         const int hs = ((const int *)(D + gather_desc_off_patt(R)))[p];
+         v4d cur[4];
+         row_of(0, cur);
+#pragma unroll
+         for (int k = 1; k < NLK; k++) {
+            v4d x[4];
+            row_of(k, x);
+            jit_mul(x, cur);
+            jit_copy(cur, x);
+         }
+         jit_root_lds(a, cur, 0.0, sPi, flag, iclass, q, hs, valid);
+      }
+      landed();
+   }
+}
+
 __global__ __launch_bounds__(256) void zpm_kernel(const unsigned char *z, long z_stride, int n_tips, int n_patt, int zw, unsigned int *out)
 {
    const long h = (long)blockIdx.x * 256 + threadIdx.x;
diff --git a/paml_amd/engine.py b/paml_amd/engine.py
--- a/paml_amd/engine.py
+++ b/paml_amd/engine.py
@@ -24,6 +24,7 @@
     "paml_amd_jit_prebuild", "paml_amd_profile", "paml_amd_profile_read", "paml_amd_counters", "paml_amd_kernel_name", "paml_amd_debug_program", "paml_amd_debug_jit",
     "paml_amd_cherry_tables", "paml_amd_debug_jit_tables",
     "paml_amd_subtree_tables", "paml_amd_subtree_order", "paml_amd_debug_subtree_order", "paml_amd_debug_subtree_classes", "paml_amd_debug_jit_subtree", "paml_amd_debug_subtree_select",
+    "paml_amd_gather_walk", "paml_amd_debug_gather_tiles",
     "paml_amd_debug_code_order", "paml_amd_debug_branch_plan",
     "paml_amd_pairset_create", "paml_amd_pairset_destroy", "paml_amd_pairset_get_counts", "paml_amd_pairset_set_pi", "paml_amd_pairset_set_pattern",
     "paml_amd_pairset_eval", "paml_amd_pairset_failed", "paml_amd_pairset_counters",
@@ -587,6 +588,13 @@
         self._chk(self._L.paml_amd_subtree_order(self._h, C.byref(use), C.byref(nc), C.byref(sec)))
         return dict(in_use=bool(use.value), n_computed=nc.value, host_seconds=sec.value)
 
+    def gather_walk(self):
+        use, nt, nr, r, nc, sec = C.c_int(), C.c_long(), C.c_long(), C.c_int(), C.c_long(), C.c_double()
+        self._L.paml_amd_gather_walk.argtypes = [C.c_void_p, C.POINTER(C.c_int), C.POINTER(C.c_long), C.POINTER(C.c_long), C.POINTER(C.c_int), C.POINTER(C.c_long),
+                                                 C.POINTER(C.c_double)]
+        self._chk(self._L.paml_amd_gather_walk(self._h, C.byref(use), C.byref(nt), C.byref(nr), C.byref(r), C.byref(nc), C.byref(sec)))
+        return dict(in_use=bool(use.value), tiles=nt.value, rows=nr.value, R=r.value, n_computed=nc.value, host_seconds=sec.value)
+
     def counters(self):
         a, b = C.c_long(), C.c_long()
         self._L.paml_amd_counters(self._h, C.byref(a), C.byref(b))
@@ -807,6 +815,38 @@
     return out
 
 
+def debug_gather_tiles(keys, bound, order=None, wflag=None, R=128):
+    L = lib()
+    keys = np.ascontiguousarray(keys, dtype=np.uint32)
+    bound = np.ascontiguousarray(bound, dtype=np.uint32)
+    nk, n_patt = keys.shape
+    order = None if order is None else np.ascontiguousarray(order, dtype=np.uint32)
+    wflag = None if wflag is None else np.ascontiguousarray(wflag, dtype=np.uint8)
+    L.paml_amd_debug_gather_tiles.argtypes = [C.c_int, C.c_void_p, C.c_void_p, C.c_void_p, C.c_void_p, C.c_long, C.c_int, C.c_void_p, C.c_long,
+                                              C.POINTER(C.c_long), C.POINTER(C.c_long)]
+    nt, nr = C.c_long(), C.c_long()
+    db = L.paml_amd_debug_gather_tiles(nk, _p(keys), _p(bound), _p(order), _p(wflag), n_patt, int(R), None, 0, C.byref(nt), C.byref(nr))
+    if db < 0:
+        raise EngineError("debug_gather_tiles failed (%d)" % db)
+    blocks = np.zeros(nt.value * db, dtype=np.uint8)
+    L.paml_amd_debug_gather_tiles(nk, _p(keys), _p(bound), _p(order), _p(wflag), n_patt, int(R), _p(blocks), blocks.size, C.byref(nt), C.byref(nr))
+    off_slot = 32 + 4 * (R + 4)
+    tiles = []
+    for t in range(nt.value):
+        d = blocks[t * db:(t + 1) * db]
+        head = d[:32].view(np.int32)
+        rows = d[32:off_slot].view(np.uint32)
+        start = [0, int(head[2]), int(head[3]), int(head[4]), int(head[5])]
+        count = int(head[1])
+        slot = d[off_slot:off_slot + 512].reshape(4, 128)
+        tiles.append(dict(first=int(head[0]), count=count, slots=int(head[5]), start=start[:nk],
+                          rows=[rows[start[k]:start[k + 1]].tolist() for k in range(nk)],
+                          slot=np.stack([slot[k, :count].astype(np.int64) - start[k] for k in range(nk)]), slot_tail=slot[:nk, count:].copy(),
+                          flag=d[off_slot + 512:off_slot + 640][:count].copy(), flag_tail=d[off_slot + 512:off_slot + 640][count:].copy(),
+                          patt=d[off_slot + 640:off_slot + 640 + 512].view(np.int32)[:count].copy()))
+    return tiles, nr.value
+
+
 def debug_subtree_select(tree, z, n_states, n_codes, K=1, scale_node=None):
     L = lib()
     ptr, flat = tree.csr()
```

Measured after the change: 4.871 billion site-patterns/s, median of 6. 1.07x the previous value.
